# TrondVQ/UncertaintyQuantification-SleepApnea-1DCNN

Hardware: AMD Instinct MI355X
Metric: 30s-windows/sec for MCD T=50 & DE M=8 inference at 1/2/4/8 MI355X (higher is better)
Workload: dtype fp32; 1 GPU; global_batch=16384, seq_len=60, parallelism=dp1, mcd_passes=50, de_members=8, bn_mode_mcd=batch

## Files before the change

### uncertaintyquantification_sleepapnea_1dcnn_amd/csrc/x3_bindings.cpp

```cpp
#include <ATen/ATen.h>
#include <c10/core/DeviceGuard.h>
#include <c10/hip/HIPStream.h>
#include <torch/library.h>

#include <hip/hip_runtime_api.h>

#include "x3_args.h"

namespace apneauq {
int x3_lds_bytes(int layer);
int x3_tile_samples(int layer);
int x3_wg_per_cu(int layer);
hipError_t x3_launch_layer(int layer, const x3::LayerArgs& A, int grid, hipStream_t stream);
hipError_t x3_launch_l1(const x3::L1Args& A, hipStream_t stream);
hipError_t x3_launch_aff(const x3::AffArgs& A, hipStream_t stream);
hipError_t x3_launch_head(const x3::HeadArgs& A, hipStream_t stream);
}

namespace {

constexpr int kCh[7] = {4, 128, 192, 224, 96, 256, 96};
constexpr int kKs[6] = {7, 5, 3, 7, 9, 9};

inline hipStream_t cur_stream() { return c10::hip::getCurrentHIPStream().stream(); }
inline void check(hipError_t e, const char* what) { TORCH_CHECK(e == hipSuccess, what, " failed: ", hipGetErrorString(e)); }

inline void need(const at::Tensor& t, at::ScalarType dt, int64_t min_numel, const char* what) {
  TORCH_CHECK(t.is_cuda() && t.scalar_type() == dt && t.is_contiguous(), what, ": contiguous GPU tensor of dtype ", dt,
              " required");
  TORCH_CHECK(t.numel() >= min_numel, what, ": ", t.numel(), " elements, need >= ", min_numel);
  TORCH_CHECK(reinterpret_cast<uintptr_t>(t.data_ptr()) % 16 == 0, what, ": 16-B alignment required");
}

int num_cus(const at::Tensor& t) {
  int n = 0;
  check(hipDeviceGetAttribute(&n, hipDeviceAttributeMultiprocessorCount, t.device().index()), "hipDeviceGetAttribute");
  return n > 0 ? n : 256;
}

void x3_layer(int64_t layer, const at::Tensor& in, at::Tensor& out, const at::Tensor& wfrag, int64_t w_gstride,
              const at::Tensor& bias, const at::Tensor& wscale, int64_t p_gstride, const at::Tensor& aff_in,
              int64_t aff_gstride, const c10::optional<at::Tensor>& stats, int64_t n_win, int64_t groups,
              bool in_shared, int64_t thr_in, int64_t thr_out, int64_t seed, int64_t pass_base,
              int64_t window_offset, int64_t grid, const c10::optional<at::Tensor>& smax_in,
              const c10::optional<at::Tensor>& amax_in, const c10::optional<at::Tensor>& smax_out,
              const c10::optional<at::Tensor>& gscale_in, bool sign_in, bool sign_out) {
  TORCH_CHECK(layer >= 1 && layer <= 5, "x3_layer: layer must be 1..5 (block 2..6)");
  TORCH_CHECK(n_win >= 1 && groups >= 1, "x3_layer: empty launch");
  const int cin = kCh[layer], cout = kCh[layer + 1], ks = kKs[layer];
  const int64_t samples = n_win * groups, samples_in = in_shared ? n_win : samples;
  const int ts = apneauq::x3_tile_samples((int)layer);
  const int64_t tpg = (n_win + ts - 1) / ts;
  TORCH_CHECK(tpg * groups < (int64_t(1) << 31), "x3_layer: too many tiles");
  const int64_t wgroups = w_gstride ? groups : 1, pgroups = p_gstride ? groups : 1;
  need(in, at::kFloat, samples_in * 60 * cin, "x3_layer: in");
  need(out, at::kFloat, layer == 5 ? samples * 2 * cout : samples * 60 * cout, "x3_layer: out");
  const int64_t frag = (int64_t)(cin / 32) * ks * (cout / 16) * 128;
  TORCH_CHECK(w_gstride == 0 || w_gstride == frag, "x3_layer: w_gstride must be 0 or ", frag);
  need(wfrag, at::kHalf, wgroups * frag * 8, "x3_layer: wfrag");
  TORCH_CHECK(p_gstride == 0 || p_gstride == cout, "x3_layer: p_gstride must be 0 or ", cout);
  need(bias, at::kFloat, pgroups * cout, "x3_layer: bias");
  need(wscale, at::kFloat, pgroups, "x3_layer: wscale");
  TORCH_CHECK(aff_gstride == 0 || aff_gstride == 2 * cin, "x3_layer: aff_gstride must be 0 or ", 2 * cin);
  need(aff_in, at::kFloat, (aff_gstride ? groups : 1) * 2 * cin, "x3_layer: aff_in");
  double* st = nullptr;
  if (stats.has_value()) {
    need(*stats, at::kDouble, groups * apneauq::x3::kStatSlots * 2 * cout, "x3_layer: stats");
    st = stats->data_ptr<double>();
  }
  TORCH_CHECK(thr_in >= 0 && thr_in <= 65536 && thr_out >= 0 && thr_out <= 65536, "x3_layer: thresholds");
  const bool pre = smax_in.has_value() && smax_in->defined();
  TORCH_CHECK(pre == (amax_in.has_value() && amax_in->defined()), "x3_layer: smax_in and amax_in go together");
  if (pre) {
    need(*smax_in, at::kInt, samples_in, "x3_layer: smax_in");
    need(*amax_in, at::kFloat, (aff_gstride ? groups : 1) * 2, "x3_layer: amax_in");
  }
  const bool gpre = gscale_in.has_value() && gscale_in->defined();
  TORCH_CHECK(!(pre && gpre), "x3_layer: per-sample and per-group prescale are exclusive");
  if (gpre) need(*gscale_in, at::kFloat, aff_gstride ? groups : 1, "x3_layer: gscale_in");
  unsigned* smo = nullptr;
  if (smax_out.has_value() && smax_out->defined()) {
    TORCH_CHECK(layer < 5, "x3_layer: block 6 feeds the fp32 head (no smax_out)");
    need(*smax_out, at::kInt, samples, "x3_layer: smax_out");
    smo = reinterpret_cast<unsigned*>(smax_out->data_ptr<int>());
  }
  const at::DeviceGuard guard(in.device());
  apneauq::x3::LayerArgs A;
  A.in = in.data_ptr<float>();
  A.out = out.data_ptr<float>();
  A.wfrag = wfrag.data_ptr();
  A.w_gstride = w_gstride;
  A.bias = bias.data_ptr<float>();
  A.wscale = wscale.data_ptr<float>();
  A.p_gstride = (int)p_gstride;
  A.aff_in = aff_in.data_ptr<float>();
  A.aff_gstride = (int)aff_gstride;
  A.stats = st;
  A.smax_in = pre ? reinterpret_cast<const unsigned*>(smax_in->data_ptr<int>()) : nullptr;
  A.amax_in = pre ? amax_in->data_ptr<float>() : nullptr;
  A.smax_out = smo;
  A.gscale_in = gpre ? gscale_in->data_ptr<float>() : nullptr;
  A.n_win = (int)n_win;
  A.groups = (int)groups;
  A.tiles_per_group = (int)tpg;
  A.total_tiles = (int)(tpg * groups);
  A.in_shared = in_shared ? 1 : 0;
  TORCH_CHECK(!(sign_in && in_shared), "x3_layer: the shared block-1 output carries no masks");
  TORCH_CHECK(!(sign_out && layer == 5), "x3_layer: block 6 reduces its masked output in place");
  A.sign_in = sign_in ? 1 : 0;
  A.sign_out = sign_out ? 1 : 0;
  A.thr_in = (unsigned)thr_in;
  A.thr_out = (unsigned)thr_out;
  A.layer = (int)layer;
  A.pass_base = (unsigned)pass_base;
  A.window_offset = (unsigned)window_offset;
  A.seed = (unsigned long long)seed;
  int g = grid > 0 ? (int)grid : num_cus(in) * apneauq::x3_wg_per_cu((int)layer);
  if (g > A.total_tiles) g = A.total_tiles;
  check(apneauq::x3_launch_layer((int)layer, A, g, cur_stream()), "x3_layer");
}

void x3_l1(const at::Tensor& x, const at::Tensor& w, const at::Tensor& b, at::Tensor& out,
           const c10::optional<at::Tensor>& stats, int64_t n_win, int64_t groups, const c10::optional<at::Tensor>& smax) {
  TORCH_CHECK(n_win >= 1 && groups >= 1, "x3_l1: empty launch");
  need(x, at::kFloat, n_win * 60 * 4, "x3_l1: x");
  need(w, at::kFloat, groups * 7 * 4 * 128, "x3_l1: w");
  need(b, at::kFloat, groups * 128, "x3_l1: b");
  need(out, at::kFloat, groups * n_win * 60 * 128, "x3_l1: out");
  double* st = nullptr;
  if (stats.has_value()) {
    need(*stats, at::kDouble, groups * apneauq::x3::kStatSlots * 2 * 128, "x3_l1: stats");
    st = stats->data_ptr<double>();
  }
  unsigned* smp = nullptr;
  if (smax.has_value() && smax->defined()) {
    need(*smax, at::kInt, groups * n_win, "x3_l1: smax");
    smp = reinterpret_cast<unsigned*>(smax->data_ptr<int>());
  }
  const int64_t bpg = (n_win + apneauq::x3::kL1Win - 1) / apneauq::x3::kL1Win;
  TORCH_CHECK(bpg * groups < (int64_t(1) << 31), "x3_l1: too many blocks");
  const at::DeviceGuard guard(x.device());
  apneauq::x3::L1Args A{x.data_ptr<float>(), w.data_ptr<float>(), b.data_ptr<float>(), out.data_ptr<float>(), st, smp,
                        (int)n_win, (int)groups, (int)bpg};
  check(apneauq::x3_launch_l1(A, cur_stream()), "x3_l1");
}

void x3_aff(const c10::optional<at::Tensor>& stats, const at::Tensor& gamma, const at::Tensor& beta, at::Tensor& mmean,
            at::Tensor& mvar, at::Tensor& aff, int64_t C, int64_t groups, int64_t p_gstride, bool update,
            int64_t repeat, double inv_count, double eps, double momentum, double dsc,
            const c10::optional<at::Tensor>& amax, const c10::optional<at::Tensor>& gscale, bool running) {
  TORCH_CHECK(C >= 1 && C <= 4096 && groups >= 1, "x3_aff: bad sizes");
  TORCH_CHECK(!(running && update), "x3_aff: running affine and the moving update are exclusive");
  TORCH_CHECK(p_gstride == 0 || p_gstride == C, "x3_aff: p_gstride must be 0 or C");
  const int64_t pg = p_gstride ? groups : 1;
  need(gamma, at::kFloat, pg * C, "x3_aff: gamma");
  need(beta, at::kFloat, pg * C, "x3_aff: beta");
  need(mmean, at::kFloat, pg * C, "x3_aff: moving_mean");
  need(mvar, at::kFloat, pg * C, "x3_aff: moving_variance");
  need(aff, at::kFloat, groups * 2 * C, "x3_aff: aff");
  const double* st = nullptr;
  if (stats.has_value()) {
    need(*stats, at::kDouble, groups * apneauq::x3::kStatSlots * 2 * C, "x3_aff: stats");
    st = stats->data_ptr<double>();
  }
  TORCH_CHECK(!update || st != nullptr, "x3_aff: the moving update needs batch moments");
  float* amp = nullptr;
  if (amax.has_value() && amax->defined()) {
    need(*amax, at::kFloat, groups * 2, "x3_aff: amax");
    amp = amax->data_ptr<float>();
  }
  float* gsp = nullptr;
  if (gscale.has_value() && gscale->defined()) {
    TORCH_CHECK(st != nullptr && amp == nullptr, "x3_aff: gscale needs batch moments and excludes amax");
    need(*gscale, at::kFloat, groups, "x3_aff: gscale");
    gsp = gscale->data_ptr<float>();
  }
  const at::DeviceGuard guard(gamma.device());
  apneauq::x3::AffArgs A{st, gamma.data_ptr<float>(), beta.data_ptr<float>(), mmean.data_ptr<float>(),
                         mvar.data_ptr<float>(), aff.data_ptr<float>(), amp, gsp, (int)C, (int)groups, (int)p_gstride,
                         update ? 1 : 0, (int)repeat, inv_count, (float)eps, (float)momentum, (float)dsc,
                         running ? 1 : 0};
  check(apneauq::x3_launch_aff(A, cur_stream()), "x3_aff");
}

void x3_head(const at::Tensor& sums, const at::Tensor& aff, int64_t aff_gstride, const at::Tensor& dw,
             const at::Tensor& db, int64_t p_gstride, at::Tensor& out, int64_t n_win, int64_t groups, bool logits) {
  const int C = kCh[6];
  const int64_t samples = n_win * groups;
  TORCH_CHECK(samples >= 1 && samples < (int64_t(1) << 31), "x3_head: bad sample count");
  TORCH_CHECK(aff_gstride == 0 || aff_gstride == 2 * C, "x3_head: aff_gstride");
  TORCH_CHECK(p_gstride == 0 || p_gstride == C, "x3_head: p_gstride");
  need(sums, at::kFloat, samples * 2 * C, "x3_head: sums");
  need(aff, at::kFloat, (aff_gstride ? groups : 1) * 2 * C, "x3_head: aff");
  need(dw, at::kFloat, (p_gstride ? groups : 1) * C, "x3_head: dense w");
  need(db, at::kFloat, p_gstride ? groups : 1, "x3_head: dense b");
  need(out, at::kFloat, samples, "x3_head: out");
  const at::DeviceGuard guard(sums.device());
  apneauq::x3::HeadArgs A{sums.data_ptr<float>(), aff.data_ptr<float>(), dw.data_ptr<float>(), db.data_ptr<float>(),
                          out.data_ptr<float>(), C, (int)n_win, (int)samples, (int)aff_gstride, (int)p_gstride,
                          logits ? 1 : 0};
  check(apneauq::x3_launch_head(A, cur_stream()), "x3_head");
}

int64_t x3_lds(int64_t layer) { return apneauq::x3_lds_bytes((int)layer); }

}

TORCH_LIBRARY_FRAGMENT(apneauq, m) {
  m.def("x3_layer(int layer, Tensor input, Tensor(a!) out, Tensor wfrag, int w_gstride, Tensor bias, Tensor wscale, "
        "int p_gstride, Tensor aff_in, int aff_gstride, Tensor(b!)? stats, int n_win, int groups, bool in_shared, "
        "int thr_in, int thr_out, int seed, int pass_base, int window_offset, int grid, Tensor? smax_in=None, "
        "Tensor? amax_in=None, Tensor(c!)? smax_out=None, Tensor? gscale_in=None, bool sign_in=False, bool sign_out=False) -> ()");
  m.def("x3_l1(Tensor x, Tensor w, Tensor b, Tensor(a!) out, Tensor(b!)? stats, int n_win, int groups, "
        "Tensor(c!)? smax=None) -> ()");
  m.def("x3_aff(Tensor? stats, Tensor gamma, Tensor beta, Tensor(a!) mmean, Tensor(b!) mvar, Tensor(c!) aff, int C, "
        "int groups, int p_gstride, bool update, int repeat, float inv_count, float eps, float momentum, float dsc, "
        "Tensor(d!)? amax=None, Tensor(e!)? gscale=None, bool running=False) -> ()");
  m.def("x3_head(Tensor sums, Tensor aff, int aff_gstride, Tensor dw, Tensor db, int p_gstride, Tensor(a!) out, "
        "int n_win, int groups, bool logits) -> ()");
  m.def("x3_lds(int layer) -> int", &x3_lds);
}

TORCH_LIBRARY_IMPL(apneauq, CUDA, m) {
  m.impl("x3_layer", &x3_layer);
  m.impl("x3_l1", &x3_l1);
  m.impl("x3_head", &x3_head);
  m.impl("x3_aff", &x3_aff);
}
```

### uncertaintyquantification_sleepapnea_1dcnn_amd/csrc/x3_layers.hip

```cpp
#include "common.h"
#include "x3_args.h"

namespace apneauq {
namespace x3 {

typedef _Float16 f16x8 __attribute__((ext_vector_type(8)));
typedef _Float16 f16x4 __attribute__((ext_vector_type(4)));
typedef _Float16 f16x2 __attribute__((ext_vector_type(2)));
typedef __attribute__((address_space(1))) const f16x8 gf16x8;

constexpr int kStagers = 4;
constexpr int kL = 60, kSR = 64, kHalo = 4;
__host__ __device__ constexpr int row_bytes(int ck) { return 4 * ck + 32; }
__device__ __forceinline__ int sample_prescale(unsigned rmax_bits, const float* amax) {
  const float b = __builtin_fmaf(amax[0], __uint_as_float(rmax_bits), amax[1]);
  int e = 0;
  if (b > 0.f && b < INFINITY) frexpf(b, &e);
  return min(100, max(-100, 14 - e));
}

__host__ __device__ constexpr int lds_rows(int S) { return kHalo + S * kSR + kHalo; }
__host__ __device__ constexpr int buf_bytes(int S, int ck) { return lds_rows(S) * row_bytes(ck); }
__host__ __device__ constexpr int lds_bytes(int S, int cout, int ck) {
  return 2 * buf_bytes(S, ck) + 2 * cout * 8 + 2 * S * 4;
}

template <typename T>
__device__ __forceinline__ T gld(const void* p) {
  return *(const __attribute__((address_space(1))) T*)(p);
}

__device__ __forceinline__ int opaque_tid() {
  int t = threadIdx.x;
  asm volatile("" : "+v"(t));
  return t;
}

__device__ __forceinline__ f32x4 mfma(const f16x8& a, const f16x8& b, const f32x4& c) {
  return __builtin_amdgcn_mfma_f32_16x16x32_f16(a, b, c, 0, 0, 0);
}

__device__ __forceinline__ void lds_barrier() {
  __builtin_amdgcn_fence(__ATOMIC_RELEASE, "workgroup", "local");
  __builtin_amdgcn_s_barrier();
  __builtin_amdgcn_fence(__ATOMIC_ACQUIRE, "workgroup", "local");
}

__device__ __forceinline__ int xcd_wg() {
  const int nwg = gridDim.x, bid = blockIdx.x;
  const int q = nwg / 8, rem = nwg % 8, xcd = bid % 8;
  return (xcd < rem ? xcd * (q + 1) : rem * (q + 1) + (xcd - rem) * q) + bid / 8;
}

template <int NW, int WPC>
constexpr int waves_per_eu() { return NW * WPC > 8 ? (NW * WPC + 3) / 4 : NW * WPC <= 4 ? 1 : 2; }
constexpr int loaders(int lw) { return lw > 0 ? lw : 0; }
template <int CIN, int COUT, int KS, int S, int WM, int WN, bool LAST, int LW, int CK, int WPC, bool PS>
__global__ __launch_bounds__((WM * WN + loaders(LW)) * 64, (waves_per_eu<WM * WN + loaders(LW), WPC>())) void layer_kernel(
    const LayerArgs A) {
  extern __shared__ __attribute__((aligned(16))) char smem[];
  constexpr int NWM = WM * WN, NW = NWM + loaders(LW), kThreads = NW * 64;
  constexpr int kCK = CK, kRowB = row_bytes(CK), NQ = CK / 32, kQ = CK / 4;
  constexpr int kS = S, kBufB = buf_bytes(S, CK), kValidRows = S * kL, kUnits = kValidRows * kQ;
  constexpr int SW = LW > 0 ? LW : LW < 0 ? (-LW < NW ? -LW : NW) : (kStagers < NW ? kStagers : NW);
  constexpr int kSBase = LW > 0 ? NWM * 64 : 0;
  constexpr int kST = SW * 64;
  constexpr int kNU = (kUnits + kST - 1) / kST;
  static_assert(kST % kQ == 0 && (CK == 32 || CK == 64), "a staging thread keeps one channel quad");
  constexpr int NCH = CIN / kCK, NCTA = COUT / 16, NCT = NCTA / WN, NRT = 4 * S / WM, PAD = (KS - 1) / 2;
  constexpr int NSTEP = NCH * NQ * KS;
  constexpr int RG = NCT >= 4                        ? 1
                     : (NCT >= 3 && NCT * NRT > 16)    ? 1
                     : NCT == 1                        ? 4
                                                       : 2;
  constexpr bool BDB = NCT * NRT <= 24 && RG < 4;
  static_assert(NRT % RG == 0, "row-tile groups");
  constexpr long long FRAG_STEP = (long long)NCTA * 128;
  static_assert(CIN % kCK == 0 && COUT % 16 == 0, "channel tiling");
  static_assert(NCTA % WN == 0 && (4 * S) % WM == 0, "wave tiling");
  static_assert(NRT % 4 == 0, "whole 64-row sample slots per wave row (epilogue keys, block 6 sums)");
  double* st = reinterpret_cast<double*>(smem + 2 * kBufB);
  float* wsc = reinterpret_cast<float*>(smem + 2 * kBufB + 2 * COUT * 8);

  const int tid = threadIdx.x, lane = tid & 63;
  const int wave = __builtin_amdgcn_readfirstlane(tid >> 6);
  const int wn = wave % WN, wm = (wave / WN) % WM;
  const int ct0 = wn * NCT, rt0 = wm * NRT;
  const int m = lane & 15, h = lane >> 4;
  APNEAUQ_DASSERT(blockDim.x == kThreads);

  for (int i = tid; i < 2 * kBufB / 16; i += kThreads) reinterpret_cast<f32x4*>(smem)[i] = f32x4{0.f, 0.f, 0.f, 0.f};
  for (int i = tid; i < 2 * COUT; i += kThreads) st[i] = 0.0;
  __syncthreads();

  const int wg = xcd_wg();
  const int tpg = (A.n_win + S - 1) / S;
  const int total_tiles = tpg * A.groups;
  const int t_begin = (int)((long long)wg * total_tiles / gridDim.x);
  const int t_end = (int)((long long)(wg + 1) * total_tiles / gridDim.x);
  if (t_begin >= t_end) return;
  const int slot = wg % kStatSlots;

  const bool loader = LW > 0 && wave >= NWM;
  const bool stager = LW > 0 ? loader : wave < SW;
  struct Stage {
    f32x4 v[kNU];
    f32x4 a, b;
  };
  Stage s0;
  const bool hash_in = A.thr_in != 0u && !A.sign_in;
  const bool sign_in = A.thr_in != 0u && A.sign_in;
  const bool prescale = PS && A.smax_in != nullptr;
  int key_tile = -1;
  unsigned skeys[kS];
  unsigned skey_tile = 0u;
  static_assert(kS <= 8, "packed per-sample exponents");
  constexpr int kSP = (kS + 3) / 4;
  unsigned sa_pack[kSP];
  auto load_chunk = [&](int tile, int c, Stage& R) {
    const int tid = opaque_tid() - kSBase, q = tid % kQ;
    const int g = tile / tpg;
    const int w0 = (tile - g * tpg) * kS;
    const float* af = A.aff_in + (long long)g * A.aff_gstride + c * kCK + 4 * q;
    R.a = gld<f32x4>(af);
    R.b = gld<f32x4>(af + CIN);
#pragma unroll
    for (int u = 0; u < kNU; ++u) {
      const int ri = tid / kQ + (kST / kQ) * u;
      R.v[u] = f32x4{-0.f, -0.f, -0.f, -0.f};
      if (ri < kValidRows) {
        const int s = ri / kL, t = ri - s * kL, w = w0 + s;
        if (w < A.n_win) {
          const long long si = A.in_shared ? w : (long long)g * A.n_win + w;
          R.v[u] = gld<f32x4>(A.in + (si * kL + t) * CIN + c * kCK + 4 * q);
        }
      }
    }
  };
  auto store_chunk = [&](int tile, int c, char* buf, const Stage& R) {
    const int tid = opaque_tid() - kSBase, q = tid % kQ;
    const int g = tile / tpg;
    const int w0 = (tile - g * tpg) * kS;
    if (tile != key_tile) {
      const unsigned skey = stream_key(A.seed, A.layer - 1, A.pass_base + g);
      skey_tile = skey;
      const float* am = A.amax_in + (A.aff_gstride ? 2 * g : 0);
      float ws0 = A.wscale[A.p_gstride ? g : 0];
      if (A.gscale_in != nullptr) ws0 *= A.gscale_in[A.aff_gstride ? g : 0];
#pragma unroll
      for (int i = 0; i < kSP; ++i) sa_pack[i] = 0u;
#pragma unroll
      for (int s = 0; s < kS; ++s) {
        skeys[s] = sample_key(skey, A.window_offset + w0 + s);
        int sa = 0;
        if (prescale && w0 + s < A.n_win) {
          const long long si = A.in_shared ? w0 + s : (long long)g * A.n_win + w0 + s;
          sa = sample_prescale(A.smax_in[si], am);
          sa_pack[s >> 2] |= ((unsigned)sa & 0xFFu) << (8 * (s & 3));
        }
        if (tid == s) wsc[(tile & 1) * kS + s] = ldexpf(ws0, -sa);
      }
      key_tile = tile;
    }
#pragma unroll
    for (int u = 0; u < kNU; ++u) {
      const int ri = tid / kQ + (kST / kQ) * u;
      if (ri >= kValidRows) continue;
      const int s = ri / kL, t = ri - s * kL, w = w0 + s;
      const f32x4 v = R.v[u];
      bool keep[4];
      if (hash_in) {
        unsigned k;
        if constexpr (!PS) {
          k = sample_key(skey_tile, A.window_offset + w);
        } else {
          k = skeys[0];
#pragma unroll
          for (int j = 1; j < kS; ++j) k = s == j ? skeys[j] : k;
        }
        const unsigned b01 = dropout_bits2(k, t, c * kCK + 4 * q);
        const unsigned b23 = dropout_bits2(k, t, c * kCK + 4 * q + 2);
        keep[0] = (b01 & 0xFFFFu) >= A.thr_in;
        keep[1] = (b01 >> 16) >= A.thr_in;
        keep[2] = (b23 & 0xFFFFu) >= A.thr_in;
        keep[3] = (b23 >> 16) >= A.thr_in;
      } else if (sign_in) {
#pragma unroll
        for (int i = 0; i < 4; ++i) keep[i] = !__builtin_signbit(v[i]);
      } else {
#pragma unroll
        for (int i = 0; i < 4; ++i) keep[i] = true;
      }
      const bool valid = w < A.n_win;
      int sa = 0;
      if (prescale) {
        unsigned sp = sa_pack[0];
#pragma unroll
        for (int i = 1; i < kSP; ++i) sp = (s >> 2) == i ? sa_pack[i] : sp;
        sa = __builtin_amdgcn_sbfe((int)sp, 8 * (s & 3), 8);
      }
      float a[4];
#pragma unroll
      for (int i = 0; i < 4; ++i) a[i] = (valid && keep[i]) ? ldexpf(__builtin_fmaf(v[i], R.a[i], R.b[i]), sa) : 0.f;
      uint2 hi, lo;
#pragma unroll
      for (int p = 0; p < 2; ++p) {
        const unsigned u = __builtin_bit_cast(unsigned, (f16x2){(_Float16)a[2 * p], (_Float16)a[2 * p + 1]});
        unsigned l;
        asm("v_fma_mixlo_f16 %0, %1, -1.0, %2 op_sel_hi:[1,0,0]" : "=v"(l) : "v"(u), "v"(a[2 * p]));
        asm("v_fma_mixhi_f16 %0, %1, -1.0, %2 op_sel:[1,0,0] op_sel_hi:[1,0,0]"
                     : "+v"(l)
                     : "v"(u), "v"(a[2 * p + 1]));
        (p ? hi.y : hi.x) = u;
        (p ? lo.y : lo.x) = l;
      }
      char* row = buf + (kHalo + s * kSR + t) * kRowB + 8 * q;
      *reinterpret_cast<uint2*>(row) = hi;
      *reinterpret_cast<uint2*>(row + 2 * kCK) = lo;
    }
  };

  f32x4 acc[NCT][NRT];
#pragma unroll
  for (int ct = 0; ct < NCT; ++ct)
#pragma unroll
    for (int rt = 0; rt < NRT; ++rt) acc[ct][rt] = f32x4{0.f, 0.f, 0.f, 0.f};
  auto wbase = [&](int tile) -> const gf16x8* {
    const int g = tile / tpg;
    return (const gf16x8*)(A.wfrag) + (long long)g * A.w_gstride + ct0 * 128 + lane;
  };
  f16x8 ah[NCT], al[NCT];
  auto load_a = [&](const gf16x8* p, f16x8 (&xh)[NCT], f16x8 (&xl)[NCT]) {
#pragma unroll
    for (int ct = 0; ct < NCT; ++ct) {
      xh[ct] = p[ct * 128];
      xl[ct] = p[ct * 128 + 64];
    }
  };

  const int bofs = ((rt0 * 16 + m + kHalo - PAD) * kRowB) + 16 * h;

  auto compute_chunk = [&](int c, const char* buf, const gf16x8* wcur, const gf16x8* wnxt, auto&& hook) {
#pragma unroll
    for (int kk = 0; kk < NQ * KS; ++kk) {
      const int q2 = kk / KS, j = kk - q2 * KS;
      const char* bb = buf + bofs + q2 * 64;
      const int s = c * NQ * KS + kk;
      const gf16x8* np = (s + 1 < NSTEP) ? wcur + (long long)(s + 1) * FRAG_STEP : wnxt;
      f16x8 nh[NCT], nl[NCT];
      load_a(np, nh, nl);
      __builtin_amdgcn_sched_barrier(0);
      auto ldb = [&](int rt, f16x8& h_, f16x8& l_) {
        h_ = *reinterpret_cast<const f16x8*>(bb + (rt * 16 + j) * kRowB);
        l_ = *reinterpret_cast<const f16x8*>(bb + (rt * 16 + j) * kRowB + 2 * kCK);
      };
      f16x8 bh[RG], bl[RG];
#pragma unroll
      for (int r = 0; r < RG; ++r) ldb(r, bh[r], bl[r]);
#pragma unroll
      for (int rg = 0; rg < NRT; rg += RG) {
        f16x8 bh2[RG], bl2[RG];
#pragma unroll
        for (int r = 0; r < RG; ++r) {
          bh2[r] = bh[r];
          bl2[r] = bl[r];
          if (BDB && rg + RG < NRT) ldb(rg + RG + r, bh2[r], bl2[r]);
          if (!BDB) ldb(rg + r, bh[r], bl[r]);
        }
        __builtin_amdgcn_sched_barrier(0);
#pragma unroll
        for (int r = 0; r < RG; ++r)
#pragma unroll
          for (int ct = 0; ct < NCT; ++ct) acc[ct][rg + r] = mfma(ah[ct], bh[r], acc[ct][rg + r]);
#pragma unroll
        for (int r = 0; r < RG; ++r)
#pragma unroll
          for (int ct = 0; ct < NCT; ++ct) acc[ct][rg + r] = mfma(al[ct], bh[r], acc[ct][rg + r]);
#pragma unroll
        for (int r = 0; r < RG; ++r)
#pragma unroll
          for (int ct = 0; ct < NCT; ++ct) acc[ct][rg + r] = mfma(ah[ct], bl[r], acc[ct][rg + r]);
#pragma unroll
        for (int r = 0; r < RG; ++r) {
          bh[r] = bh2[r];
          bl[r] = bl2[r];
        }
      }
#pragma unroll
      for (int ct = 0; ct < NCT; ++ct) {
        ah[ct] = nh[ct];
        al[ct] = nl[ct];
      }
      __builtin_amdgcn_sched_barrier(0);
      if (kk == (NQ * KS) / 2) hook();
    }
  };

  auto epilogue = [&](int tile) {
    const int lane = opaque_tid() & 63, m = lane & 15, h = lane >> 4;
    const int g = tile / tpg;
    const int w0 = (tile - g * tpg) * kS;
    float wsq[NRT / 4];
#pragma unroll
    for (int q = 0; q < NRT / 4; ++q) wsq[q] = wsc[(tile & 1) * kS + (rt0 >> 2) + q];
    const bool track = PS && !LAST && A.smax_out != nullptr;
    float mxs[NRT / 4];
#pragma unroll
    for (int q = 0; q < NRT / 4; ++q) mxs[q] = 0.f;
    const float* bias = A.bias + (long long)g * A.p_gstride;
    const bool drop = (LAST || A.sign_out) && A.thr_out != 0u;
    unsigned skeys[NRT / 4];
    if (drop) {
      const unsigned skey = stream_key(A.seed, A.layer, A.pass_base + g);
#pragma unroll
      for (int q = 0; q < NRT / 4; ++q)
        skeys[q] = sample_key(skey, A.window_offset + w0 + (rt0 >> 2) + q);
    }
#pragma unroll
    for (int ct = 0; ct < NCT; ++ct) {
      const int co0 = (ct0 + ct) * 16 + 4 * h;
      const f32x4 b4 = gld<f32x4>(bias + co0);
      f32x4 s1 = {0.f, 0.f, 0.f, 0.f}, s2 = s1, k1 = s1, k0 = s1;
#pragma unroll
      for (int rt = 0; rt < NRT; ++rt) {
        const int s = (rt0 + rt) >> 2, t = (((rt0 + rt) & 3) << 4) + m, w = w0 + s;
        const bool valid = t < kL && w < A.n_win;
        f32x4 r;
#pragma unroll
        for (int e = 0; e < 4; ++e) r[e] = fmaxf(__builtin_fmaf(acc[ct][rt][e], wsq[rt >> 2], b4[e]), 0.f);
        acc[ct][rt] = f32x4{0.f, 0.f, 0.f, 0.f};
        bool keep[4] = {true, true, true, true};
        if (drop) {
          const unsigned key = skeys[rt >> 2];
          const unsigned b01 = dropout_bits2(key, t, co0), b23 = dropout_bits2(key, t, co0 + 2);
          keep[0] = (b01 & 0xFFFFu) >= A.thr_out;
          keep[1] = (b01 >> 16) >= A.thr_out;
          keep[2] = (b23 & 0xFFFFu) >= A.thr_out;
          keep[3] = (b23 >> 16) >= A.thr_out;
        }
        if (valid) {
#pragma unroll
          for (int e = 0; e < 4; ++e) {
            s1[e] += r[e];
            s2[e] = __builtin_fmaf(r[e], r[e], s2[e]);
            if (!LAST) mxs[rt >> 2] = fmaxf(mxs[rt >> 2], r[e]);
            if constexpr (LAST) {
              k1[e] += keep[e] ? r[e] : 0.f;
              k0[e] += keep[e] ? 1.f : 0.f;
            }
          }
          if constexpr (!LAST) {
            const long long sample = (long long)g * A.n_win + w;
            f32x4 o = r;
            if (drop) {
#pragma unroll
              for (int e = 0; e < 4; ++e) o[e] = keep[e] ? r[e] : __builtin_copysignf(r[e], -1.f);
            }
            *reinterpret_cast<f32x4*>(A.out + (sample * kL + t) * COUT + co0) = o;
          }
        }
        if constexpr (LAST) {
          if ((rt & 3) == 3) {
#pragma unroll
            for (int e = 0; e < 4; ++e) {
              k1[e] = group16_sum(k1[e]);
              k0[e] = group16_sum(k0[e]);
            }
            const int wl = w0 + (rt0 + rt) / 4;
            if (m == 0 && wl < A.n_win) {
              float* o = A.out + ((long long)g * A.n_win + wl) * (2 * COUT);
              *reinterpret_cast<f32x4*>(o + co0) = k1;
              *reinterpret_cast<f32x4*>(o + COUT + co0) = k0;
            }
            k1 = f32x4{0.f, 0.f, 0.f, 0.f};
            k0 = k1;
          }
        }
      }
      if (A.stats != nullptr) {
#pragma unroll
        for (int e = 0; e < 4; ++e) {
          const float a = group16_sum(s1[e]), b = group16_sum(s2[e]);
          if (m == 0) {
            atomicAdd(&st[co0 + e], (double)a);
            atomicAdd(&st[COUT + co0 + e], (double)b);
          }
        }
      }
    }
    if (track) {
#pragma unroll
      for (int q = 0; q < NRT / 4; ++q) {
        const float mq = wave_max(mxs[q]);
        const int w = w0 + (rt0 >> 2) + q;
        if (lane == 0 && w < A.n_win) atomicMax(A.smax_out + (long long)g * A.n_win + w, __float_as_uint(mq));
      }
    }
  };

  auto flush_stats = [&](int g) {
    __syncthreads();
    if (A.stats != nullptr) {
      double* dst = A.stats + ((long long)g * kStatSlots + slot) * 2 * COUT;
      for (int i = tid; i < 2 * COUT; i += kThreads) {
        atomicAdd(dst + i, st[i]);
        st[i] = 0.0;
      }
    }
    __syncthreads();
  };

  const int total = (t_end - t_begin) * NCH;
  auto chunk_tile = [&](int it) { return t_begin + it / NCH; };
  int g_cur = t_begin / tpg;
  if constexpr (LW > 0) {
    if (loader) {
      if (stager) {
        load_chunk(t_begin, 0, s0);
        store_chunk(t_begin, 0, smem, s0);
      }
      lds_barrier();
      if (stager && total > 1) load_chunk(chunk_tile(1), 1 % NCH, s0);
#pragma unroll 1
      for (int it = 0; it < total; ++it) {
        const int tile = chunk_tile(it), c = it - (tile - t_begin) * NCH;
        if (c == 0) {
          const int g = tile / tpg;
          if (g != g_cur) {
            flush_stats(g_cur);
            g_cur = g;
          }
        }
        if (stager && it + 1 < total) store_chunk(chunk_tile(it + 1), (it + 1) % NCH, smem + ((it + 1) & 1) * kBufB, s0);
        lds_barrier();
        if (stager && it + 2 < total) load_chunk(chunk_tile(it + 2), (it + 2) % NCH, s0);
      }
      flush_stats(g_cur);
      return;
    }
    lds_barrier();
    load_a(wbase(t_begin), ah, al);
#pragma unroll 1
    for (int it = 0; it < total; ++it) {
      const int tile = chunk_tile(it), c = it - (tile - t_begin) * NCH;
      if (c == 0) {
        const int g = tile / tpg;
        if (g != g_cur) {
          flush_stats(g_cur);
          g_cur = g;
        }
      }
      const gf16x8* wcur = wbase(tile);
      const gf16x8* wnxt = wbase(tile + 1 < t_end ? tile + 1 : tile);
      compute_chunk(c, smem + (it & 1) * kBufB, wcur, wnxt, []() {});
      if (c == NCH - 1) epilogue(tile);
      lds_barrier();
    }
    flush_stats(g_cur);
    return;
  }
  if (stager) {
    load_chunk(t_begin, 0, s0);
    store_chunk(t_begin, 0, smem, s0);
  }
  lds_barrier();
  if (stager && total > 1) load_chunk(chunk_tile(1), 1 % NCH, s0);
  load_a(wbase(t_begin), ah, al);
#pragma unroll 1
  for (int it = 0; it < total; ++it) {
    const int tile = chunk_tile(it), c = it - (tile - t_begin) * NCH;
    if (c == 0) {
      const int g = tile / tpg;
      if (g != g_cur) {
        flush_stats(g_cur);
        g_cur = g;
      }
    }
    const gf16x8* wcur = wbase(tile);
    const gf16x8* wnxt = wbase(tile + 1 < t_end ? tile + 1 : tile);
    char* buf = smem + (it & 1) * kBufB;
    char* nbuf = smem + ((it + 1) & 1) * kBufB;
    compute_chunk(c, buf, wcur, wnxt, [&]() {
      if (stager && it + 1 < total) store_chunk(chunk_tile(it + 1), (it + 1) % NCH, nbuf, s0);
    });
    if (c == NCH - 1) epilogue(tile);
    lds_barrier();
    if (stager && it + 2 < total) load_chunk(chunk_tile(it + 2), (it + 2) % NCH, s0);
  }
  flush_stats(g_cur);
}

__global__ __launch_bounds__(256) void l1_kernel(const L1Args A) {
  __shared__ float xs[kL1Win][kL + 6][4];
  __shared__ float red[2][2][128];
  __shared__ unsigned wmax[kL1Win];
  const int g = blockIdx.x / A.blocks_per_group;
  const int w0 = (blockIdx.x - g * A.blocks_per_group) * kL1Win;
  const int tid = threadIdx.x, c = tid & 127, half = tid >> 7;
  for (int i = tid; i < kL1Win * (kL + 6) * 4; i += 256) {
    const int s = i / ((kL + 6) * 4), r = (i / 4) % (kL + 6), ci = i & 3;
    const int t = r - 3, w = w0 + s;
    xs[s][r][ci] = (t >= 0 && t < kL && w < A.n_win) ? A.x[((long long)w * kL + t) * 4 + ci] : 0.f;
  }
  float wr[7][4];
#pragma unroll
  for (int j = 0; j < 7; ++j)
#pragma unroll
    for (int ci = 0; ci < 4; ++ci) wr[j][ci] = A.w[(((long long)g * 7 + j) * 4 + ci) * 128 + c];
  const float bc = A.b[g * 128 + c];
  if (tid < kL1Win) wmax[tid] = 0u;
  __syncthreads();
  float s1 = 0.f, s2 = 0.f;
  for (int s = 0; s < kL1Win; ++s) {
    const int w = w0 + s;
    if (w >= A.n_win) break;
    float* o = A.out + (((long long)g * A.n_win + w) * kL) * 128 + c;
    float mx = 0.f;
    for (int t = half * 30; t < half * 30 + 30; ++t) {
      float v = bc;
#pragma unroll
      for (int j = 0; j < 7; ++j)
#pragma unroll
        for (int ci = 0; ci < 4; ++ci) v = __builtin_fmaf(xs[s][t + j][ci], wr[j][ci], v);
      v = fmaxf(v, 0.f);
      o[t * 128] = v;
      s1 += v;
      s2 = __builtin_fmaf(v, v, s2);
      mx = fmaxf(mx, v);
    }
    if (A.smax != nullptr) {
      mx = wave_max(mx);
      if ((tid & 63) == 0) atomicMax(&wmax[s], __float_as_uint(mx));
    }
  }
  if (A.stats != nullptr || A.smax != nullptr) {
    red[half][0][c] = s1;
    red[half][1][c] = s2;
    __syncthreads();
    if (A.stats != nullptr && tid < 128) {
      double* dst = A.stats + ((long long)g * kStatSlots + (blockIdx.x % kStatSlots)) * 2 * 128;
      atomicAdd(dst + c, (double)red[0][0][c] + (double)red[1][0][c]);
      atomicAdd(dst + 128 + c, (double)red[0][1][c] + (double)red[1][1][c]);
    }
    if (A.smax != nullptr && tid < kL1Win && w0 + tid < A.n_win) A.smax[(long long)g * A.n_win + w0 + tid] = wmax[tid];
  }
}

__device__ __forceinline__ void aff_moments(const AffArgs& A, int g, int c, float& mean, float& var) {
  const double* p = A.stats + (long long)g * kStatSlots * 2 * A.C + c;
  double a = 0.0, b = 0.0;
#pragma unroll
  for (int s = 0; s < kStatSlots; ++s) {
    a += p[s * 2 * A.C];
    b += p[s * 2 * A.C + A.C];
  }
  const double mu = a * A.inv_count;
  mean = (float)mu;
  var = (float)fmax(b * A.inv_count - mu * mu, 0.0);
}

__global__ __launch_bounds__(256) void aff_kernel(const AffArgs A) {
  __shared__ float red[2][4];
  const int tid = threadIdx.x;
  if ((int)blockIdx.x == A.groups) {
    for (int c = tid; c < A.C; c += 256)
      for (int g = 0; g < A.groups; ++g) {
        const long long po = (long long)g * A.p_gstride + c;
        float mean, var;
        aff_moments(A, g, c, mean, var);
        for (int r = 0; r < A.repeat; ++r) {
          A.mmean[po] = A.mmean[po] * A.momentum + mean * (1.f - A.momentum);
          A.mvar[po] = A.mvar[po] * A.momentum + var * (1.f - A.momentum);
        }
      }
    return;
  }
  {
    const int g = blockIdx.x;
    float ms = 0.f, mt = 0.f;
    for (int c = tid; c < A.C; c += 256) {
      const long long po = (long long)g * A.p_gstride + c;
      float mean, var;
      if (A.stats != nullptr && !A.running) {
        aff_moments(A, g, c, mean, var);
      } else {
        mean = A.mmean[po];
        var = A.mvar[po];
      }
      const float sc = A.gamma[po] / sqrtf(var + A.eps);
      const float s_ = sc * A.dsc, t_ = (A.beta[po] - mean * sc) * A.dsc;
      A.aff[((long long)g * 2) * A.C + c] = s_;
      A.aff[((long long)g * 2 + 1) * A.C + c] = t_;
      if (A.gscale != nullptr) {
        const double* p = A.stats + (long long)g * kStatSlots * 2 * A.C + A.C + c;
        double q = 0.0;
        for (int s = 0; s < kStatSlots; ++s) q += p[s * 2 * A.C];
        ms = fmaxf(ms, __builtin_fmaf(fabsf(s_), (float)sqrt(fmax(q, 0.0)) * 1.0001f, fabsf(t_)));
      } else {
        ms = fmaxf(ms, fabsf(s_));
        mt = fmaxf(mt, fabsf(t_));
      }
    }
    if (A.gscale != nullptr) {
      ms = wave_max(ms);
      if ((tid & 63) == 0) red[0][tid >> 6] = ms;
      __syncthreads();
      const float bnd = fmaxf(fmaxf(red[0][0], red[0][1]), fmaxf(red[0][2], red[0][3]));
      int e = 0;
      if (bnd > 0.f && bnd < INFINITY) frexpf(bnd, &e);
      const int sa = min(100, max(-100, 14 - e));
      for (int c = tid; c < A.C; c += 256) {
        float* af = A.aff + (long long)g * 2 * A.C + c;
        af[0] = ldexpf(af[0], sa);
        af[A.C] = ldexpf(af[A.C], sa);
      }
      if (tid == 0) A.gscale[g] = ldexpf(1.f, -sa);
      return;
    }
    if (A.amax == nullptr) return;
    ms = wave_max(ms);
    mt = wave_max(mt);
    if ((tid & 63) == 0) {
      red[0][tid >> 6] = ms;
      red[1][tid >> 6] = mt;
    }
    __syncthreads();
    if (tid == 0) {
      A.amax[2 * g] = fmaxf(fmaxf(red[0][0], red[0][1]), fmaxf(red[0][2], red[0][3]));
      A.amax[2 * g + 1] = fmaxf(fmaxf(red[1][0], red[1][1]), fmaxf(red[1][2], red[1][3]));
    }
  }
}

__global__ __launch_bounds__(256) void head_kernel(const HeadArgs A) {
  const int lane = threadIdx.x & 63;
  const long long sidx = (long long)blockIdx.x * 4 + (threadIdx.x >> 6);
  if (sidx >= A.samples) return;
  const int g = (int)(sidx / A.n_win);
  const float* s = A.sums + sidx * 2 * A.C;
  const float* af = A.aff + (long long)g * A.aff_gstride;
  const float* dw = A.dw + (long long)g * A.p_gstride;
  float v = 0.f;
  for (int c = lane; c < A.C; c += 64) v += dw[c] * __builtin_fmaf(af[c], s[c], af[A.C + c] * s[A.C + c]);
  v = wave_sum(v);
  if (lane == 0) {
    const float logit = v * (1.0f / kL) + A.db[A.p_gstride ? g : 0];
    A.out[sidx] = A.out_logits ? logit : 1.0f / (1.0f + expf(-logit));
  }
}

template <int CIN, int COUT, int KS, int S, int WM, int WN, bool LAST, int LW, int CK, int WPC, bool PS>
hipError_t launch_layer(const LayerArgs& A, int grid, hipStream_t stream) {
  constexpr int lds = lds_bytes(S, COUT, CK);
  static_assert(WPC * lds <= 160 * 1024, "LDS of the workgroups sharing a CU");
  auto k = layer_kernel<CIN, COUT, KS, S, WM, WN, LAST, LW, CK, WPC, PS>;
  static bool attr = false;
  if (!attr) {
    hipError_t e = hipFuncSetAttribute(reinterpret_cast<const void*>(k), hipFuncAttributeMaxDynamicSharedMemorySize, lds);
    if (e != hipSuccess) return e;
    attr = true;
  }
  hipLaunchKernelGGL(k, dim3(grid), dim3((WM * WN + loaders(LW)) * 64), lds, stream, A);
  return hipGetLastError();
}

}

#ifdef APNEAUQ_X3_TABLE
#include APNEAUQ_X3_TABLE
#else
#define APNEAUQ_X3_LAYERS(X)                     \
  X(1, 128, 192, 5, 4, 2, 4, false, -8, 0, 32, 1) \
  X(2, 192, 224, 3, 2, 1, 7, false, 4, 4, 64, 1) \
  X(3, 224, 96, 7, 4, 2, 2, false, 4, 4, 32, 1)  \
  X(4, 96, 256, 9, 2, 1, 8, false, 4, 4, 32, 1)  \
  X(5, 256, 96, 9, 4, 2, 2, true, 4, 4, 64, 1)
#endif

int x3_lds_bytes(int layer) {
#define APNEAUQ_X3_LDS(L, CI, CO, K, S, WM, WN, LAST, LW, LWB, CK, WPC) \
  if (layer == L) return x3::lds_bytes(S, CO, CK);
  APNEAUQ_X3_LAYERS(APNEAUQ_X3_LDS)
#undef APNEAUQ_X3_LDS
  return 0;
}

int x3_tile_samples(int layer) {
#define APNEAUQ_X3_TS(L, CI, CO, K, S, WM, WN, LAST, LW, LWB, CK, WPC) \
  if (layer == L) return S;
  APNEAUQ_X3_LAYERS(APNEAUQ_X3_TS)
#undef APNEAUQ_X3_TS
  return 0;
}

int x3_wg_per_cu(int layer) {
#define APNEAUQ_X3_WPC(L, CI, CO, K, S, WM, WN, LAST, LW, LWB, CK, WPC) \
  if (layer == L) return WPC;
  APNEAUQ_X3_LAYERS(APNEAUQ_X3_WPC)
#undef APNEAUQ_X3_WPC
  return 1;
}

hipError_t x3_launch_layer(int layer, const x3::LayerArgs& A, int grid, hipStream_t stream) {
  using namespace x3;
  const bool ps = A.smax_in != nullptr || A.smax_out != nullptr;
#define APNEAUQ_X3_LAUNCH(L, CI, CO, K, S, WM, WN, LAST, LW, LWB, CK, WPC)                                  \
  if (layer == L) {                                                                                       \
    return ps ? launch_layer<CI, CO, K, S, WM, WN, LAST, LW, CK, WPC, true>(A, grid, stream)               \
              : launch_layer<CI, CO, K, S, WM, WN, LAST, LWB, CK, WPC, false>(A, grid, stream);            \
  }
  APNEAUQ_X3_LAYERS(APNEAUQ_X3_LAUNCH)
#undef APNEAUQ_X3_LAUNCH
  return hipErrorInvalidValue;
}

hipError_t x3_launch_l1(const x3::L1Args& A, hipStream_t stream) {
  const int grid = A.groups * A.blocks_per_group;
  if (grid <= 0) return hipSuccess;
  hipLaunchKernelGGL(x3::l1_kernel, dim3(grid), dim3(256), 0, stream, A);
  return hipGetLastError();
}

hipError_t x3_launch_aff(const x3::AffArgs& A, hipStream_t stream) {
  const int blocks = A.groups + (A.stats != nullptr && A.update ? 1 : 0);
  hipLaunchKernelGGL(x3::aff_kernel, dim3(blocks), dim3(256), 0, stream, A);
  return hipGetLastError();
}

hipError_t x3_launch_head(const x3::HeadArgs& A, hipStream_t stream) {
  if (A.samples <= 0) return hipSuccess;
  hipLaunchKernelGGL(x3::head_kernel, dim3((A.samples + 3) / 4), dim3(256), 0, stream, A);
  return hipGetLastError();
}

}
```

### uncertaintyquantification_sleepapnea_1dcnn_amd/ops/x3.py

```python
from __future__ import annotations

import math
import os
from typing import Callable, Dict, List, Optional, Sequence

import torch

from ..models.spec import ModelSpec
from . import _ext, fused, rng

CH = fused.FUSED_CHANNELS
KS = fused.FUSED_KSIZES
STAT_SLOTS = 16
TILE = 4
CK = 32
BYTES_PER_SAMPLE = 60 * (192 + 256) * 4
R1_BYTES = 60 * 128 * 4


def supports(spec: ModelSpec) -> bool:
    return fused.supports(spec)


def pack_conv(kernel: torch.Tensor):
    k, cin, cout = kernel.shape
    assert cin % CK == 0 and cout % 16 == 0
    w = kernel.detach().to(torch.float64)
    amax = float(w.abs().max()) if w.numel() else 0.0
    sw = 13 - math.frexp(amax)[1] + 1 if amax > 0 else 0
    ws = (w * (2.0 ** sw)).float()
    hi = ws.half()
    lo = (ws - hi.float()).half()
    nch, nct = cin // CK, cout // 16

    def frag(p):
        v = p.reshape(k, nch, 4, 8, nct, 16)
        return v.permute(1, 0, 4, 2, 5, 3).reshape(nch, k, nct, 64, 8)

    fr = torch.stack([frag(hi), frag(lo)], dim=3)
    return fr.contiguous().reshape(-1), 2.0 ** (-sw)


def unpack_conv(fr: torch.Tensor, wscale: float, k: int, cin: int, cout: int) -> torch.Tensor:
    nch, nct = cin // CK, cout // 16
    v = fr.reshape(nch, k, nct, 2, 4, 16, 8).float()
    w = v[:, :, :, 0] + v[:, :, :, 1]
    w = w.permute(1, 0, 3, 5, 2, 4).reshape(k, cin, cout)
    return w.double().mul(wscale).float()


class X3Model:

    def __init__(self, spec: ModelSpec, params: Sequence[Dict[str, torch.Tensor]], device=None):
        if not supports(spec):
            raise ValueError("the x3 engine implements the reference (60, 4) no-pool architecture")
        self.spec = spec
        self.G = len(params)
        dev = torch.device(device) if device is not None else params[0]["conv1d_1/kernel"].device
        if dev.type == "cuda" and dev.index is None:
            dev = torch.device("cuda", torch.cuda.current_device())
        self.device = dev
        f32 = dict(dtype=torch.float32, device=dev)
        self.w1 = torch.stack([p["conv1d_1/kernel"].to(**f32) for p in params]).contiguous()
        self.b1 = torch.stack([p["conv1d_1/bias"].to(**f32) for p in params]).contiguous()
        self.wfrag: List[Optional[torch.Tensor]] = [None]
        self.wscale: List[Optional[torch.Tensor]] = [None]
        self.bias: List[torch.Tensor] = [self.b1]
        for l in range(1, 6):
            frs, scs = [], []
            for p in params:
                fr, sc = pack_conv(p[f"conv1d_{l + 1}/kernel"].to(dev))
                frs.append(fr)
                scs.append(sc)
            self.wfrag.append(torch.stack(frs).contiguous())
            self.wscale.append(torch.tensor(scs, **f32))
            self.bias.append(torch.stack([p[f"conv1d_{l + 1}/bias"].to(**f32) for p in params]).contiguous())
        self.bn = []
        for l in range(6):
            names = [f"batchnorm_{l + 1}/{n}" for n in ("gamma", "beta", "moving_mean", "moving_variance")]
            entry = []
            for n in names:
                src = params[0][n]
                if self.G == 1 and src.device == dev and src.dtype == torch.float32 and src.is_contiguous():
                    entry.append(src.view(1, -1))
                else:
                    entry.append(torch.stack([p[n].to(**f32) for p in params]).contiguous())
            self.bn.append(entry)
        self.dw = torch.stack([p["output_layer/kernel"].to(**f32).reshape(-1) for p in params]).contiguous()
        self.db = torch.stack([p["output_layer/bias"].to(**f32).reshape(-1) for p in params]).reshape(-1).contiguous()
        self._ws: Dict[tuple, "_Workspace"] = {}

    def workspace(self, samples: int, n_r1: int, groups: int) -> "_Workspace":
        ws = self._ws.get("ws")
        if ws is None or ws.samples < samples or ws.n_r1 < n_r1 or ws.groups < groups:
            self._ws.clear()
            ws = self._ws["ws"] = _Workspace(self.device, samples, n_r1, groups)
        return ws


class _Workspace:
    def __init__(self, dev, samples: int, n_r1: int, groups: int):
        self.samples, self.n_r1, self.groups = int(samples), int(n_r1), max(int(groups), 1)
        f32 = dict(dtype=torch.float32, device=dev)
        self.r1 = torch.empty(n_r1 * 60 * CH[1], **f32)
        self.buf = [torch.empty(samples * 60 * 192, **f32), torch.empty(samples * 60 * 256, **f32)]
        self.sums = torch.empty(samples * 2 * CH[6], **f32)
        self.out = torch.empty(samples, **f32)
        self.stats = [torch.zeros(max(groups, 1) * STAT_SLOTS * 2 * CH[l + 1], dtype=torch.float64, device=dev)
                      for l in range(6)]
        self.aff = [torch.empty(max(groups, 1) * 2 * CH[l + 1], **f32) for l in range(6)]
        self.smax = [torch.zeros(n_r1 if l == 0 else samples, dtype=torch.int32, device=dev) for l in range(5)]
        self.amax = [torch.zeros(max(groups, 1) * 2, **f32) for l in range(6)]
        self.gscale = [torch.ones(max(groups, 1), **f32) for l in range(5)] + [None]

    def smax_out(self, l: int, k: int) -> Optional[torch.Tensor]:
        if l >= 5:
            return None
        return self.smax[l][:k].zero_()


def _ops():
    return _ext.ops()


_SIGN_DEFAULT = "2,4"


def _sign_layers() -> frozenset:
    v = os.environ.get("APNEAUQ_X3_SIGN_MASK", _SIGN_DEFAULT)
    return frozenset(int(t) for t in v.replace(" ", "").split(",") if t)


def _sign(l: int, sl: frozenset):
    return (l - 1) in sl and l >= 2, l in sl and l <= 4


def _dsc(rate: float) -> float:
    return 1.0 / (1.0 - rate) if rate < 1.0 else 0.0


def _sync_stats(sync: Callable, st: torch.Tensor, groups: int, c: int) -> None:
    v = st[: groups * STAT_SLOTS * 2 * c].view(groups, STAT_SLOTS, 2 * c)
    tot = v.sum(1)
    sync(tot)
    v.zero_()
    v[:, 0].copy_(tot)


def _max_samples(dev, per_sample: int, frac: float = 0.45) -> int:
    import os

    free = torch.cuda.mem_get_info(dev)[0]
    cap = float(os.environ.get("APNEAUQ_X3_WS_GB", "20")) * 2 ** 30
    return max(1, int(min(free * frac, cap)) // per_sample)


@torch.no_grad()
def mcd_batch(model: X3Model, x: torch.Tensor, n_pass: int, seed: int, pass_base: int = 0, window_offset: int = 0,
              update_moving: bool = True, sync: Optional[Callable] = None, global_n: Optional[int] = None,
              max_samples: Optional[int] = None, grid: int = 0) -> torch.Tensor:
    assert model.G == 1, "mcd_batch runs one model"
    spec, o = model.spec, _ops()
    x = x.to(device=model.device, dtype=torch.float32).contiguous()
    n = x.shape[0]
    gn = int(global_n or n)
    if max_samples is None:
        max_samples = _max_samples(model.device, BYTES_PER_SAMPLE + R1_BYTES)
        if sync is not None:
            t = torch.tensor([float(max_samples)], dtype=torch.float64, device=model.device)
            import torch.distributed as dist

            from ..parallel import comm

            comm.run("chunking_all_reduce_min", t, lambda: dist.all_reduce(t, op=dist.ReduceOp.MIN))
            max_samples = int(t.item())
    ref_n = n
    if sync is not None and global_n:
        import torch.distributed as dist

        w = dist.get_world_size() if dist.is_initialized() else 1
        ref_n = -(-gn // w)
    if ref_n > max_samples:
        return _mcd_batch_windowed(model, x, n_pass, seed, pass_base, window_offset, update_moving, sync, gn,
                                   max_samples)
    cap = max(1, min(n_pass, max_samples // max(ref_n, 1)))
    n_chunks = -(-n_pass // cap)
    chunk = -(-n_pass // n_chunks)
    ws = model.workspace(chunk * n, n, chunk)
    inv_count = 1.0 / (gn * 60.0)
    thr = [rng.dropout_threshold(b.dropout) for b in spec.blocks]
    dsc = [_dsc(b.dropout) for b in spec.blocks]
    eps, mom = float(spec.bn_epsilon), float(spec.bn_momentum)
    seed = int(seed) & ((1 << 63) - 1)
    sl = _sign_layers()
    out = torch.empty(n_pass, n, dtype=torch.float32, device=model.device)
    ws.stats[0].zero_()
    o.x3_l1(x, model.w1, model.b1, ws.r1, ws.stats[0], n, 1, None)
    if sync is not None:
        _sync_stats(sync, ws.stats[0], 1, CH[1])
    g, b, mm, mv = model.bn[0]
    o.x3_aff(ws.stats[0], g, b, mm, mv, ws.aff[0], CH[1], 1, 0, bool(update_moving), n_pass, inv_count, eps, mom, dsc[0],
             None, ws.gscale[0])
    for t0 in range(0, n_pass, chunk):
        tc = min(chunk, n_pass - t0)
        pb = int(pass_base) + t0
        for l in range(1, 6):
            c = CH[l + 1]
            st = ws.stats[l]
            st[: tc * STAT_SLOTS * 2 * c].zero_()
            src = ws.r1 if l == 1 else ws.buf[(l - 2) % 2]
            dst = ws.sums if l == 5 else ws.buf[(l - 1) % 2]
            o.x3_layer(l, src, dst, model.wfrag[l], 0, model.bias[l], model.wscale[l], 0, ws.aff[l - 1],
                       0 if l == 1 else 2 * CH[l], st, n, tc, l == 1, thr[l - 1], thr[l], seed, pb,
                       int(window_offset), int(grid), None, None, None, ws.gscale[l - 1], *_sign(l, sl))
            if sync is not None:
                _sync_stats(sync, st, tc, c)
            g, b, mm, mv = model.bn[l]
            o.x3_aff(st, g, b, mm, mv, ws.aff[l], c, tc, 0, bool(update_moving), 1, inv_count, eps, mom, dsc[l],
                     None, ws.gscale[l])
        o.x3_head(ws.sums, ws.aff[5], 2 * CH[6], model.dw, model.db, 0, ws.out, n, tc, False)
        out[t0: t0 + tc].copy_(ws.out[: tc * n].view(tc, n))
    return out


def _mcd_batch_windowed(model: X3Model, x: torch.Tensor, n_pass: int, seed: int, pass_base: int,
                        window_offset: int, update_moving: bool, sync: Optional[Callable], gn: int,
                        max_samples: int) -> torch.Tensor:
    spec, o = model.spec, _ops()
    n = x.shape[0]
    wc = max(1, int(max_samples))
    bounds = [(s, min(n, s + wc)) for s in range(0, n, wc)]
    ws = model.workspace(wc, wc, 1)
    inv_count = 1.0 / (gn * 60.0)
    thr = [rng.dropout_threshold(b.dropout) for b in spec.blocks]
    dsc = [_dsc(b.dropout) for b in spec.blocks]
    eps, mom = float(spec.bn_epsilon), float(spec.bn_momentum)
    seed = int(seed) & ((1 << 63) - 1)
    sl = _sign_layers()
    out = torch.empty(n_pass, n, dtype=torch.float32, device=model.device)

    def run(s: int, e: int, upto: int, pb: int, stats_layer: int) -> None:
        m = e - s
        o.x3_l1(x[s:e], model.w1, model.b1, ws.r1, ws.stats[0] if stats_layer == 0 else None, m, 1, None)
        for l in range(1, upto + 1):
            src = ws.r1 if l == 1 else ws.buf[(l - 2) % 2]
            dst = ws.sums if l == 5 else ws.buf[(l - 1) % 2]
            o.x3_layer(l, src, dst, model.wfrag[l], 0, model.bias[l], model.wscale[l], 0, ws.aff[l - 1],
                       0 if l == 1 else 2 * CH[l], ws.stats[l] if l == stats_layer else None, m, 1, l == 1,
                       thr[l - 1], thr[l], seed, pb, int(window_offset) + s, 0, None, None, None, ws.gscale[l - 1],
                       *_sign(l, sl))

    def finish_layer(l: int, repeat: int) -> None:
        if sync is not None:
            _sync_stats(sync, ws.stats[l], 1, CH[l + 1])
        g, b, mm, mv = model.bn[l]
        o.x3_aff(ws.stats[l], g, b, mm, mv, ws.aff[l], CH[l + 1], 1, 0, bool(update_moving), repeat, inv_count, eps,
                 mom, dsc[l], None, ws.gscale[l])

    ws.stats[0].zero_()
    for s, e in bounds:
        run(s, e, 0, int(pass_base), 0)
    finish_layer(0, n_pass)
    for t in range(n_pass):
        pb = int(pass_base) + t
        for l in range(1, 6):
            ws.stats[l].zero_()
            for s, e in bounds:
                run(s, e, l, pb, l)
            finish_layer(l, 1)
        for s, e in bounds:
            run(s, e, 5, pb, -1)
            o.x3_head(ws.sums, ws.aff[5], 0, model.dw, model.db, 0, ws.out, e - s, 1, False)
            out[t, s:e].copy_(ws.out[: e - s])
    return out


@torch.no_grad()
def forward_running(model: X3Model, x: torch.Tensor, n_pass: int = 1, dropout: bool = False, seed: int = 0,
                    pass_offset: int = 0, window_offset: int = 0, logits: bool = False,
                    max_samples: Optional[int] = None) -> torch.Tensor:
    x = x.to(device=model.device, dtype=torch.float32).contiguous()
    n = x.shape[0]
    groups = (n_pass if dropout else model.G) if n > 0 else 1
    if max_samples is None:
        max_samples = _max_samples(model.device, BYTES_PER_SAMPLE + R1_BYTES)
    wc = max(1, int(max_samples) // max(groups, 1))
    if n <= wc:
        return _forward_running(model, x, n_pass, dropout, seed, pass_offset, window_offset, logits)
    parts = [_forward_running(model, x[s: s + wc], n_pass, dropout, seed, pass_offset, int(window_offset) + s, logits)
             for s in range(0, n, wc)]
    return torch.cat(parts, dim=2)


def _forward_running(model: X3Model, x: torch.Tensor, n_pass: int, dropout: bool, seed: int, pass_offset: int,
                     window_offset: int, logits: bool) -> torch.Tensor:
    spec, o = model.spec, _ops()
    n = x.shape[0]
    G = model.G
    if dropout and G != 1:
        raise ValueError("MC Dropout runs one model")
    if not dropout:
        n_pass = 1
    groups = n_pass if dropout else G
    ws = model.workspace(groups * n, n * G, max(groups, G))
    thr = [rng.dropout_threshold(b.dropout) if dropout else 0 for b in spec.blocks]
    dsc = [_dsc(b.dropout) if dropout else 1.0 for b in spec.blocks]
    eps, mom = float(spec.bn_epsilon), float(spec.bn_momentum)
    seed = int(seed) & ((1 << 63) - 1)
    if not dropout:
        return _predict_members(model, ws, x, G, eps, mom, logits)
    sl = _sign_layers()
    for l in range(6):
        g, b, mm, mv = model.bn[l]
        o.x3_aff(None, g, b, mm, mv, ws.aff[l], CH[l + 1], G, CH[l + 1] if G > 1 else 0, False, 1, 1.0, eps, mom,
                 dsc[l], ws.amax[l])
    o.x3_l1(x, model.w1, model.b1, ws.r1, None, n, G, ws.smax[0])
    per_member = G > 1
    for l in range(1, 6):
        src = ws.r1 if l == 1 else ws.buf[(l - 2) % 2]
        dst = ws.sums if l == 5 else ws.buf[(l - 1) % 2]
        wstride = model.wfrag[l].shape[1] // 8 if per_member else 0
        sm = ws.smax_out(l, groups * n)
        o.x3_layer(l, src, dst, model.wfrag[l], wstride, model.bias[l], model.wscale[l],
                   CH[l + 1] if per_member else 0, ws.aff[l - 1], 2 * CH[l] if per_member else 0, None, n, groups,
                   dropout and l == 1, thr[l - 1], thr[l], seed, int(pass_offset),
                   int(window_offset), 0, ws.smax[l - 1], ws.amax[l - 1], sm, None, *_sign(l, sl))
    o.x3_head(ws.sums, ws.aff[5], 2 * CH[6] if per_member else 0, model.dw, model.db, CH[6] if per_member else 0,
              ws.out, n, groups, bool(logits))
    return ws.out[: groups * n].view(G, n_pass, n).clone()


def _predict_members(model: X3Model, ws: "_Workspace", x: torch.Tensor, G: int, eps: float, mom: float,
                     logits: bool) -> torch.Tensor:
    spec, o = model.spec, _ops()
    n = x.shape[0]
    per_member = G > 1
    ps = CH[1:] if per_member else [0] * 6
    o.zero_buffers([ws.stats[l][: G * STAT_SLOTS * 2 * CH[l + 1]] for l in range(5)])
    g, b, mm, mv = model.bn[5]
    o.x3_aff(None, g, b, mm, mv, ws.aff[5], CH[6], G, ps[5], False, 1, 1.0, eps, mom, 1.0, None)
    o.x3_l1(x, model.w1, model.b1, ws.r1, ws.stats[0], n, G, None)
    for l in range(1, 6):
        g, b, mm, mv = model.bn[l - 1]
        o.x3_aff(ws.stats[l - 1], g, b, mm, mv, ws.aff[l - 1], CH[l], G, ps[l - 1], False, 1, 1.0, eps, mom, 1.0,
                 None, ws.gscale[l - 1], True)
        src = ws.r1 if l == 1 else ws.buf[(l - 2) % 2]
        dst = ws.sums if l == 5 else ws.buf[(l - 1) % 2]
        wstride = model.wfrag[l].shape[1] // 8 if per_member else 0
        o.x3_layer(l, src, dst, model.wfrag[l], wstride, model.bias[l], model.wscale[l], ps[l],
                   ws.aff[l - 1], 2 * CH[l] if per_member else 0, ws.stats[l] if l < 5 else None, n, G, False, 0, 0,
                   0, 0, 0, 0, None, None, None, ws.gscale[l - 1], False, False)
    o.x3_head(ws.sums, ws.aff[5], 2 * CH[6] if per_member else 0, model.dw, model.db, CH[6] if per_member else 0,
              ws.out, n, G, bool(logits))
    return ws.out[: G * n].view(G, 1, n).clone()


def split_f16(a: torch.Tensor):
    hi = a.half()
    lo = (a - hi.float()).half()
    return hi, lo


def emulate_conv(h: torch.Tensor, fr: torch.Tensor, wscale: float, k: int, cin: int, cout: int) -> torch.Tensor:
    from ..models.reference import conv1d_same

    nch, nct = cin // CK, cout // 16
    v = fr.reshape(nch, k, nct, 2, 4, 16, 8).double()
    whi = v[:, :, :, 0].permute(1, 0, 3, 5, 2, 4).reshape(k, cin, cout)
    wlo = v[:, :, :, 1].permute(1, 0, 3, 5, 2, 4).reshape(k, cin, cout)
    ah, al = split_f16(h.float())
    ah, al = ah.double(), al.double()
    z = torch.zeros(cout, dtype=torch.float64)
    y = conv1d_same(ah, whi, z) + conv1d_same(ah, wlo, z) + conv1d_same(al, whi, z)
    return y * wscale
```

Baseline: 62120 windows/s.

## Add dense-row tiling for conv blocks 2-5 that packs timesteps across window boundaries

Adds a dense-row variant of the conv layer kernel. Each tile covers a contiguous run of timestep rows across windows (64*S rows), instead of S whole 60-step windows padded to 64-row slots. This removes the wasted MFMA rows that come from padding each 60-step window to 64. The cost is extra staging of halo edges, per-row slot arithmetic, and more complex dropout key and mask handling in the epilogue. It is enabled by default for layers 1-4 in the batch-moment and ensemble paths.

```diff
diff --git a/uncertaintyquantification_sleepapnea_1dcnn_amd/csrc/x3_bindings.cpp b/uncertaintyquantification_sleepapnea_1dcnn_amd/csrc/x3_bindings.cpp
--- a/uncertaintyquantification_sleepapnea_1dcnn_amd/csrc/x3_bindings.cpp
+++ b/uncertaintyquantification_sleepapnea_1dcnn_amd/csrc/x3_bindings.cpp
@@ -6,12 +6,14 @@
 #include <hip/hip_runtime_api.h>
 
 #include "x3_args.h"
+#include "x3_dense_map.h"
 
 namespace apneauq {
 int x3_lds_bytes(int layer);
 int x3_tile_samples(int layer);
 int x3_wg_per_cu(int layer);
-hipError_t x3_launch_layer(int layer, const x3::LayerArgs& A, int grid, hipStream_t stream);
+bool x3_has_dense(int layer);
+hipError_t x3_launch_layer(int layer, const x3::LayerArgs& A, int grid, bool dense_rows, hipStream_t stream);
 hipError_t x3_launch_l1(const x3::L1Args& A, hipStream_t stream);
 hipError_t x3_launch_aff(const x3::AffArgs& A, hipStream_t stream);
 hipError_t x3_launch_head(const x3::HeadArgs& A, hipStream_t stream);
@@ -44,13 +46,16 @@
               bool in_shared, int64_t thr_in, int64_t thr_out, int64_t seed, int64_t pass_base,
               int64_t window_offset, int64_t grid, const c10::optional<at::Tensor>& smax_in,
               const c10::optional<at::Tensor>& amax_in, const c10::optional<at::Tensor>& smax_out,
-              const c10::optional<at::Tensor>& gscale_in, bool sign_in, bool sign_out) {
+              const c10::optional<at::Tensor>& gscale_in, bool sign_in, bool sign_out, bool dense_rows) {
   TORCH_CHECK(layer >= 1 && layer <= 5, "x3_layer: layer must be 1..5 (block 2..6)");
   TORCH_CHECK(n_win >= 1 && groups >= 1, "x3_layer: empty launch");
   const int cin = kCh[layer], cout = kCh[layer + 1], ks = kKs[layer];
   const int64_t samples = n_win * groups, samples_in = in_shared ? n_win : samples;
   const int ts = apneauq::x3_tile_samples((int)layer);
-  const int64_t tpg = (n_win + ts - 1) / ts;
+  TORCH_CHECK(!dense_rows || apneauq::x3_has_dense((int)layer), "x3_layer: layer ", layer,
+              " has no dense-row kernel");
+  TORCH_CHECK(!dense_rows || n_win < (int64_t(1) << 24), "x3_layer: too many windows for dense rows");
+  const int64_t tpg = dense_rows ? apneauq::x3::dense::tiles(n_win, 64 * ts) : (n_win + ts - 1) / ts;
   TORCH_CHECK(tpg * groups < (int64_t(1) << 31), "x3_layer: too many tiles");
   const int64_t wgroups = w_gstride ? groups : 1, pgroups = p_gstride ? groups : 1;
   need(in, at::kFloat, samples_in * 60 * cin, "x3_layer: in");
@@ -75,6 +80,8 @@
     need(*smax_in, at::kInt, samples_in, "x3_layer: smax_in");
     need(*amax_in, at::kFloat, (aff_gstride ? groups : 1) * 2, "x3_layer: amax_in");
   }
+  TORCH_CHECK(!(dense_rows && (pre || (smax_out.has_value() && smax_out->defined()))),
+              "x3_layer: the per-sample prescale kernels keep whole-window slots");
   const bool gpre = gscale_in.has_value() && gscale_in->defined();
   TORCH_CHECK(!(pre && gpre), "x3_layer: per-sample and per-group prescale are exclusive");
   if (gpre) need(*gscale_in, at::kFloat, aff_gstride ? groups : 1, "x3_layer: gscale_in");
@@ -117,7 +124,7 @@
   A.seed = (unsigned long long)seed;
   int g = grid > 0 ? (int)grid : num_cus(in) * apneauq::x3_wg_per_cu((int)layer);
   if (g > A.total_tiles) g = A.total_tiles;
-  check(apneauq::x3_launch_layer((int)layer, A, g, cur_stream()), "x3_layer");
+  check(apneauq::x3_launch_layer((int)layer, A, g, dense_rows, cur_stream()), "x3_layer");
 }
 
 void x3_l1(const at::Tensor& x, const at::Tensor& w, const at::Tensor& b, at::Tensor& out,
@@ -203,6 +210,7 @@
 }
 
 int64_t x3_lds(int64_t layer) { return apneauq::x3_lds_bytes((int)layer); }
+bool x3_has_dense(int64_t layer) { return apneauq::x3_has_dense((int)layer); }
 
 }
 
@@ -210,7 +218,8 @@
   m.def("x3_layer(int layer, Tensor input, Tensor(a!) out, Tensor wfrag, int w_gstride, Tensor bias, Tensor wscale, "
         "int p_gstride, Tensor aff_in, int aff_gstride, Tensor(b!)? stats, int n_win, int groups, bool in_shared, "
         "int thr_in, int thr_out, int seed, int pass_base, int window_offset, int grid, Tensor? smax_in=None, "
-        "Tensor? amax_in=None, Tensor(c!)? smax_out=None, Tensor? gscale_in=None, bool sign_in=False, bool sign_out=False) -> ()");
+        "Tensor? amax_in=None, Tensor(c!)? smax_out=None, Tensor? gscale_in=None, bool sign_in=False, bool sign_out=False, "
+        "bool dense_rows=False) -> ()");
   m.def("x3_l1(Tensor x, Tensor w, Tensor b, Tensor(a!) out, Tensor(b!)? stats, int n_win, int groups, "
         "Tensor(c!)? smax=None) -> ()");
   m.def("x3_aff(Tensor? stats, Tensor gamma, Tensor beta, Tensor(a!) mmean, Tensor(b!) mvar, Tensor(c!) aff, int C, "
@@ -219,6 +228,7 @@
   m.def("x3_head(Tensor sums, Tensor aff, int aff_gstride, Tensor dw, Tensor db, int p_gstride, Tensor(a!) out, "
         "int n_win, int groups, bool logits) -> ()");
   m.def("x3_lds(int layer) -> int", &x3_lds);
+  m.def("x3_has_dense(int layer) -> bool", &x3_has_dense);
 }
 
 TORCH_LIBRARY_IMPL(apneauq, CUDA, m) {
diff --git a/uncertaintyquantification_sleepapnea_1dcnn_amd/csrc/x3_dense_map.h b/uncertaintyquantification_sleepapnea_1dcnn_amd/csrc/x3_dense_map.h
--- /dev/null
+++ b/uncertaintyquantification_sleepapnea_1dcnn_amd/csrc/x3_dense_map.h
@@ -0,0 +1,41 @@
+#pragma once
+
+#ifndef __host__
+#define APNEAUQ_X3_DENSE_MAP_PLAIN 1
+#define __host__
+#define __device__
+#endif
+
+namespace apneauq {
+namespace x3 {
+namespace dense {
+
+constexpr int kLen = 60, kSlot = 64, kHaloRows = 4;
+
+__host__ __device__ constexpr long long tiles(long long n_win, int rows) { return (kLen * n_win + rows - 1) / rows; }
+__host__ __device__ constexpr int max_windows(int rows) { return (kLen - 4 + rows - 1) / kLen + 1; }
+__host__ __device__ constexpr int lds_rows(int rows) { return kHaloRows + kSlot * max_windows(rows) + kHaloRows; }
+
+__host__ __device__ constexpr long long first_row(long long tl, int rows) { return tl * rows; }
+__host__ __device__ constexpr int first_window(long long tl, int rows) { return (int)(first_row(tl, rows) / kLen); }
+__host__ __device__ constexpr int offset(long long tl, int rows) { return (int)(first_row(tl, rows) % kLen); }
+__host__ __device__ constexpr int windows(int off, int rows) { return (off + rows - 1) / kLen + 1; }
+
+__host__ __device__ constexpr int slot_of(int dl) { return (int)(((unsigned)dl & 1023u) * 1093u >> 16); }
+__host__ __device__ constexpr int step_of(int dl) { return dl - kLen * slot_of(dl); }
+__host__ __device__ constexpr int lds_row(int dl) { return kHaloRows + dl + (kSlot - kLen) * slot_of(dl); }
+
+__host__ __device__ constexpr int staged_units(int rows, int pad) { return rows + 2 * pad; }
+__host__ __device__ constexpr bool staged(int dl, int off, int rows, int pad) {
+  return dl >= 0 && dl >= off - pad && dl < off + rows + pad && dl < kLen * windows(off, rows);
+}
+
+}
+}
+}
+
+#ifdef APNEAUQ_X3_DENSE_MAP_PLAIN
+#undef __host__
+#undef __device__
+#undef APNEAUQ_X3_DENSE_MAP_PLAIN
+#endif
diff --git a/uncertaintyquantification_sleepapnea_1dcnn_amd/csrc/x3_layers.hip b/uncertaintyquantification_sleepapnea_1dcnn_amd/csrc/x3_layers.hip
--- a/uncertaintyquantification_sleepapnea_1dcnn_amd/csrc/x3_layers.hip
+++ b/uncertaintyquantification_sleepapnea_1dcnn_amd/csrc/x3_layers.hip
@@ -1,5 +1,6 @@
 #include "common.h"
 #include "x3_args.h"
+#include "x3_dense_map.h"
 
 namespace apneauq {
 namespace x3 {
@@ -21,8 +22,8 @@
 
 __host__ __device__ constexpr int lds_rows(int S) { return kHalo + S * kSR + kHalo; }
 __host__ __device__ constexpr int buf_bytes(int S, int ck) { return lds_rows(S) * row_bytes(ck); }
-__host__ __device__ constexpr int lds_bytes(int S, int cout, int ck) {
-  return 2 * buf_bytes(S, ck) + 2 * cout * 8 + 2 * S * 4;
+__host__ __device__ constexpr int lds_bytes(int S, int cout, int ck, bool dense_rows = false) {
+  return 2 * (dense_rows ? dense::lds_rows(kSR * S) * row_bytes(ck) : buf_bytes(S, ck)) + 2 * cout * 8 + 2 * S * 4;
 }
 
 template <typename T>
@@ -55,19 +56,24 @@
 template <int NW, int WPC>
 constexpr int waves_per_eu() { return NW * WPC > 8 ? (NW * WPC + 3) / 4 : NW * WPC <= 4 ? 1 : 2; }
 constexpr int loaders(int lw) { return lw > 0 ? lw : 0; }
-template <int CIN, int COUT, int KS, int S, int WM, int WN, bool LAST, int LW, int CK, int WPC, bool PS>
+template <int CIN, int COUT, int KS, int S, int WM, int WN, bool LAST, int LW, int CK, int WPC, bool PS, bool DENSE = false>
 __global__ __launch_bounds__((WM * WN + loaders(LW)) * 64, (waves_per_eu<WM * WN + loaders(LW), WPC>())) void layer_kernel(
     const LayerArgs A) {
   extern __shared__ __attribute__((aligned(16))) char smem[];
   constexpr int NWM = WM * WN, NW = NWM + loaders(LW), kThreads = NW * 64;
   constexpr int kCK = CK, kRowB = row_bytes(CK), NQ = CK / 32, kQ = CK / 4;
-  constexpr int kS = S, kBufB = buf_bytes(S, CK), kValidRows = S * kL, kUnits = kValidRows * kQ;
+  constexpr int PAD = (KS - 1) / 2, kRows = kSR * S;
+  static_assert(!DENSE || (!PS && !LAST), "dense rows: batch-moment blocks 2..5 only");
+  constexpr int kS = S, kBufB = DENSE ? dense::lds_rows(kRows) * kRowB : buf_bytes(S, CK);
+  constexpr int kValidRows = DENSE ? kRows : S * kL, kUnits = kValidRows * kQ;
   constexpr int SW = LW > 0 ? LW : LW < 0 ? (-LW < NW ? -LW : NW) : (kStagers < NW ? kStagers : NW);
   constexpr int kSBase = LW > 0 ? NWM * 64 : 0;
   constexpr int kST = SW * 64;
-  constexpr int kNU = (kUnits + kST - 1) / kST;
+  constexpr int kMainU = (kUnits + kST - 1) / kST, kNU = kMainU + (DENSE ? 1 : 0);
+  constexpr int kEdgeWaves = (2 * PAD * kQ + 63) / 64;
+  static_assert(!DENSE || (kUnits % kST == 0 && kEdgeWaves <= SW), "dense rows: whole staging steps per tile");
   static_assert(kST % kQ == 0 && (CK == 32 || CK == 64), "a staging thread keeps one channel quad");
-  constexpr int NCH = CIN / kCK, NCTA = COUT / 16, NCT = NCTA / WN, NRT = 4 * S / WM, PAD = (KS - 1) / 2;
+  constexpr int NCH = CIN / kCK, NCTA = COUT / 16, NCT = NCTA / WN, NRT = 4 * S / WM;
   constexpr int NSTEP = NCH * NQ * KS;
   constexpr int RG = NCT >= 4                        ? 1
                      : (NCT >= 3 && NCT * NRT > 16)    ? 1
@@ -94,7 +100,7 @@
   __syncthreads();
 
   const int wg = xcd_wg();
-  const int tpg = (A.n_win + S - 1) / S;
+  const int tpg = DENSE ? (int)dense::tiles(A.n_win, kRows) : (A.n_win + S - 1) / S;
   const int total_tiles = tpg * A.groups;
   const int t_begin = (int)((long long)wg * total_tiles / gridDim.x);
   const int t_end = (int)((long long)(wg + 1) * total_tiles / gridDim.x);
@@ -103,6 +109,16 @@
 
   const bool loader = LW > 0 && wave >= NWM;
   const bool stager = LW > 0 ? loader : wave < SW;
+  const bool edge_wave = DENSE && wave >= kSBase / 64 && wave - kSBase / 64 < kEdgeWaves;
+  auto dense_unit = [&](int u, int tid, int off, int& dl) -> bool {
+    const int r = tid / kQ;
+    if (u < kMainU) {
+      dl = off + r + (kST / kQ) * u;
+      return true;
+    }
+    dl = r < PAD ? off - PAD + r : off + kRows - PAD + r;
+    return edge_wave && r < 2 * PAD && dense::staged(dl, off, kRows, PAD);
+  };
   struct Stage {
     f32x4 v[kNU];
     f32x4 a, b;
@@ -120,7 +136,7 @@
   auto load_chunk = [&](int tile, int c, Stage& R) {
     const int tid = opaque_tid() - kSBase, q = tid % kQ;
     const int g = tile / tpg;
-    const int w0 = (tile - g * tpg) * kS;
+    const int w0 = (tile - g * tpg) * (DENSE ? kRows : kS);
     const float* af = A.aff_in + (long long)g * A.aff_gstride + c * kCK + 4 * q;
     R.a = gld<f32x4>(af);
     R.b = gld<f32x4>(af + CIN);
@@ -128,7 +144,14 @@
     for (int u = 0; u < kNU; ++u) {
       const int ri = tid / kQ + (kST / kQ) * u;
       R.v[u] = f32x4{-0.f, -0.f, -0.f, -0.f};
-      if (ri < kValidRows) {
+      if constexpr (DENSE) {
+        const int wf = w0 / kL, off = w0 - wf * kL;
+        int dl;
+        if (dense_unit(u, tid, off, dl) && wf + dense::slot_of(dl) < A.n_win) {
+          const long long r0 = (A.in_shared ? 0ll : (long long)g * A.n_win * kL) + wf * kL;
+          R.v[u] = gld<f32x4>(A.in + (r0 + dl) * CIN + c * kCK + 4 * q);
+        }
+      } else if (ri < kValidRows) {
         const int s = ri / kL, t = ri - s * kL, w = w0 + s;
         if (w < A.n_win) {
           const long long si = A.in_shared ? w : (long long)g * A.n_win + w;
@@ -140,7 +163,7 @@
   auto store_chunk = [&](int tile, int c, char* buf, const Stage& R) {
     const int tid = opaque_tid() - kSBase, q = tid % kQ;
     const int g = tile / tpg;
-    const int w0 = (tile - g * tpg) * kS;
+    const int w0 = (tile - g * tpg) * (DENSE ? kRows : kS);
     if (tile != key_tile) {
       const unsigned skey = stream_key(A.seed, A.layer - 1, A.pass_base + g);
       skey_tile = skey;
@@ -149,8 +172,9 @@
       if (A.gscale_in != nullptr) ws0 *= A.gscale_in[A.aff_gstride ? g : 0];
 #pragma unroll
       for (int i = 0; i < kSP; ++i) sa_pack[i] = 0u;
-#pragma unroll
-      for (int s = 0; s < kS; ++s) {
+      if (DENSE && tid == 0) wsc[(tile & 1) * kS] = ws0;
+#pragma unroll
+      for (int s = 0; s < (DENSE ? 0 : kS); ++s) {
         skeys[s] = sample_key(skey, A.window_offset + w0 + s);
         int sa = 0;
         if (prescale && w0 + s < A.n_win) {
@@ -165,8 +189,16 @@
 #pragma unroll
     for (int u = 0; u < kNU; ++u) {
       const int ri = tid / kQ + (kST / kQ) * u;
-      if (ri >= kValidRows) continue;
-      const int s = ri / kL, t = ri - s * kL, w = w0 + s;
+      int s, t, w, lrow;
+      if constexpr (DENSE) {
+        const int wf = w0 / kL, off = w0 - wf * kL;
+        int dl;
+        if (!dense_unit(u, tid, off, dl)) continue;
+        s = dense::slot_of(dl), t = dl - s * kL, w = wf + s, lrow = dense::lds_row(dl);
+      } else {
+        if (ri >= kValidRows) continue;
+        s = ri / kL, t = ri - s * kL, w = w0 + s, lrow = kHalo + s * kSR + t;
+      }
       const f32x4 v = R.v[u];
       bool keep[4];
       if (hash_in) {
@@ -214,7 +246,7 @@
         (p ? hi.y : hi.x) = u;
         (p ? lo.y : lo.x) = l;
       }
-      char* row = buf + (kHalo + s * kSR + t) * kRowB + 8 * q;
+      char* row = buf + lrow * kRowB + 8 * q;
       *reinterpret_cast<uint2*>(row) = hi;
       *reinterpret_cast<uint2*>(row + 2 * kCK) = lo;
     }
@@ -240,7 +272,13 @@
 
   const int bofs = ((rt0 * 16 + m + kHalo - PAD) * kRowB) + 16 * h;
 
-  auto compute_chunk = [&](int c, const char* buf, const gf16x8* wcur, const gf16x8* wnxt, auto&& hook) {
+  auto compute_chunk = [&](int c, int off, const char* buf, const gf16x8* wcur, const gf16x8* wnxt, auto&& hook) {
+    const char* bp[DENSE ? NRT : 1];
+    if constexpr (DENSE) {
+#pragma unroll
+      for (int rt = 0; rt < NRT; ++rt)
+        bp[rt] = buf + bofs + (off + (dense::kSlot - kL) * ((off + (rt0 + rt) * 16 + m) / kL)) * kRowB;
+    }
 #pragma unroll
     for (int kk = 0; kk < NQ * KS; ++kk) {
       const int q2 = kk / KS, j = kk - q2 * KS;
@@ -251,8 +289,9 @@
       load_a(np, nh, nl);
       __builtin_amdgcn_sched_barrier(0);
       auto ldb = [&](int rt, f16x8& h_, f16x8& l_) {
-        h_ = *reinterpret_cast<const f16x8*>(bb + (rt * 16 + j) * kRowB);
-        l_ = *reinterpret_cast<const f16x8*>(bb + (rt * 16 + j) * kRowB + 2 * kCK);
+        const char* br = DENSE ? bp[rt] + q2 * 64 : bb;
+        h_ = *reinterpret_cast<const f16x8*>(br + (rt * 16 + j) * kRowB);
+        l_ = *reinterpret_cast<const f16x8*>(br + (rt * 16 + j) * kRowB + 2 * kCK);
       };
       f16x8 bh[RG], bl[RG];
 #pragma unroll
@@ -299,39 +338,55 @@
   auto epilogue = [&](int tile) {
     const int lane = opaque_tid() & 63, m = lane & 15, h = lane >> 4;
     const int g = tile / tpg;
-    const int w0 = (tile - g * tpg) * kS;
+    const int w0 = (tile - g * tpg) * (DENSE ? kRows : kS);
     float wsq[NRT / 4];
 #pragma unroll
-    for (int q = 0; q < NRT / 4; ++q) wsq[q] = wsc[(tile & 1) * kS + (rt0 >> 2) + q];
+    for (int q = 0; q < NRT / 4; ++q) wsq[q] = wsc[(tile & 1) * kS + (DENSE ? 0 : (rt0 >> 2) + q)];
     const bool track = PS && !LAST && A.smax_out != nullptr;
     float mxs[NRT / 4];
 #pragma unroll
     for (int q = 0; q < NRT / 4; ++q) mxs[q] = 0.f;
     const float* bias = A.bias + (long long)g * A.p_gstride;
     const bool drop = (LAST || A.sign_out) && A.thr_out != 0u;
-    unsigned skeys[NRT / 4];
+    constexpr int NKEY = DENSE ? dense::max_windows(kRows) : NRT / 4;
+    const int wf = DENSE ? w0 / kL : 0, off = DENSE ? w0 - wf * kL : 0;
+    unsigned skeys[NKEY];
     if (drop) {
       const unsigned skey = stream_key(A.seed, A.layer, A.pass_base + g);
 #pragma unroll
-      for (int q = 0; q < NRT / 4; ++q)
-        skeys[q] = sample_key(skey, A.window_offset + w0 + (rt0 >> 2) + q);
+      for (int q = 0; q < NKEY; ++q)
+        skeys[q] = DENSE ? __builtin_amdgcn_readfirstlane(sample_key(skey, A.window_offset + wf + q))
+                         : sample_key(skey, A.window_offset + w0 + (rt0 >> 2) + q);
     }
 #pragma unroll
     for (int ct = 0; ct < NCT; ++ct) {
       const int co0 = (ct0 + ct) * 16 + 4 * h;
       const f32x4 b4 = gld<f32x4>(bias + co0);
       f32x4 s1 = {0.f, 0.f, 0.f, 0.f}, s2 = s1, k1 = s1, k0 = s1;
+      int mo = m;
+      if constexpr (DENSE) asm volatile("" : "+v"(mo));
 #pragma unroll
       for (int rt = 0; rt < NRT; ++rt) {
-        const int s = (rt0 + rt) >> 2, t = (((rt0 + rt) & 3) << 4) + m, w = w0 + s;
-        const bool valid = t < kL && w < A.n_win;
+        int t, w, sl = 0;
+        bool valid;
+        if constexpr (DENSE) {
+          const int dl = off + (rt0 + rt) * 16 + mo;
+          sl = dense::slot_of(dl), w = wf + sl, t = dl - sl * kL, valid = w < A.n_win;
+        } else {
+          const int s = (rt0 + rt) >> 2;
+          t = (((rt0 + rt) & 3) << 4) + m, w = w0 + s, valid = t < kL && w < A.n_win;
+        }
         f32x4 r;
 #pragma unroll
         for (int e = 0; e < 4; ++e) r[e] = fmaxf(__builtin_fmaf(acc[ct][rt][e], wsq[rt >> 2], b4[e]), 0.f);
         acc[ct][rt] = f32x4{0.f, 0.f, 0.f, 0.f};
         bool keep[4] = {true, true, true, true};
         if (drop) {
-          const unsigned key = skeys[rt >> 2];
+          unsigned key = skeys[DENSE ? 0 : rt >> 2];
+          if constexpr (DENSE) {
+#pragma unroll
+            for (int q = 1; q < NKEY; ++q) key = sl == q ? skeys[q] : key;
+          }
           const unsigned b01 = dropout_bits2(key, t, co0), b23 = dropout_bits2(key, t, co0 + 2);
           keep[0] = (b01 & 0xFFFFu) >= A.thr_out;
           keep[1] = (b01 >> 16) >= A.thr_out;
@@ -412,6 +467,7 @@
 
   const int total = (t_end - t_begin) * NCH;
   auto chunk_tile = [&](int it) { return t_begin + it / NCH; };
+  auto tile_off = [&](int tile) { return DENSE ? (int)((long long)(tile % tpg) * kRows % kL) : 0; };
   int g_cur = t_begin / tpg;
   if constexpr (LW > 0) {
     if (loader) {
@@ -452,7 +508,7 @@
       }
       const gf16x8* wcur = wbase(tile);
       const gf16x8* wnxt = wbase(tile + 1 < t_end ? tile + 1 : tile);
-      compute_chunk(c, smem + (it & 1) * kBufB, wcur, wnxt, []() {});
+      compute_chunk(c, tile_off(tile), smem + (it & 1) * kBufB, wcur, wnxt, []() {});
       if (c == NCH - 1) epilogue(tile);
       lds_barrier();
     }
@@ -480,7 +536,7 @@
     const gf16x8* wnxt = wbase(tile + 1 < t_end ? tile + 1 : tile);
     char* buf = smem + (it & 1) * kBufB;
     char* nbuf = smem + ((it + 1) & 1) * kBufB;
-    compute_chunk(c, buf, wcur, wnxt, [&]() {
+    compute_chunk(c, tile_off(tile), buf, wcur, wnxt, [&]() {
       if (stager && it + 1 < total) store_chunk(chunk_tile(it + 1), (it + 1) % NCH, nbuf, s0);
     });
     if (c == NCH - 1) epilogue(tile);
@@ -649,11 +705,11 @@
   }
 }
 
-template <int CIN, int COUT, int KS, int S, int WM, int WN, bool LAST, int LW, int CK, int WPC, bool PS>
+template <int CIN, int COUT, int KS, int S, int WM, int WN, bool LAST, int LW, int CK, int WPC, bool PS, bool DENSE = false>
 hipError_t launch_layer(const LayerArgs& A, int grid, hipStream_t stream) {
-  constexpr int lds = lds_bytes(S, COUT, CK);
+  constexpr int lds = lds_bytes(S, COUT, CK, DENSE);
   static_assert(WPC * lds <= 160 * 1024, "LDS of the workgroups sharing a CU");
-  auto k = layer_kernel<CIN, COUT, KS, S, WM, WN, LAST, LW, CK, WPC, PS>;
+  auto k = layer_kernel<CIN, COUT, KS, S, WM, WN, LAST, LW, CK, WPC, PS, DENSE>;
   static bool attr = false;
   if (!attr) {
     hipError_t e = hipFuncSetAttribute(reinterpret_cast<const void*>(k), hipFuncAttributeMaxDynamicSharedMemorySize, lds);
@@ -664,21 +720,30 @@
   return hipGetLastError();
 }
 
+template <bool HAVE, int CIN, int COUT, int KS, int S, int WM, int WN, int LW, int CK, int WPC>
+hipError_t launch_dense(const LayerArgs& A, int grid, hipStream_t stream) {
+  if constexpr (HAVE) {
+    return launch_layer<CIN, COUT, KS, S, WM, WN, false, (LW > 0 ? LW : -(WM * WN)), CK, WPC, false, true>(A, grid, stream);
+  } else {
+    return hipErrorInvalidValue;
+  }
+}
+
 }
 
 #ifdef APNEAUQ_X3_TABLE
 #include APNEAUQ_X3_TABLE
 #else
-#define APNEAUQ_X3_LAYERS(X)                     \
-  X(1, 128, 192, 5, 4, 2, 4, false, -8, 0, 32, 1) \
-  X(2, 192, 224, 3, 2, 1, 7, false, 4, 4, 64, 1) \
-  X(3, 224, 96, 7, 4, 2, 2, false, 4, 4, 32, 1)  \
-  X(4, 96, 256, 9, 2, 1, 8, false, 4, 4, 32, 1)  \
-  X(5, 256, 96, 9, 4, 2, 2, true, 4, 4, 64, 1)
+#define APNEAUQ_X3_LAYERS(X)                           \
+  X(1, 128, 192, 5, 4, 2, 4, false, -8, 0, 32, 1, true) \
+  X(2, 192, 224, 3, 2, 1, 7, false, 4, 4, 64, 1, true)  \
+  X(3, 224, 96, 7, 4, 2, 2, false, 4, 4, 32, 1, true)   \
+  X(4, 96, 256, 9, 2, 1, 8, false, 4, 4, 32, 1, true)   \
+  X(5, 256, 96, 9, 4, 2, 2, true, 4, 4, 64, 1, false)
 #endif
 
 int x3_lds_bytes(int layer) {
-#define APNEAUQ_X3_LDS(L, CI, CO, K, S, WM, WN, LAST, LW, LWB, CK, WPC) \
+#define APNEAUQ_X3_LDS(L, CI, CO, K, S, WM, WN, LAST, LW, LWB, CK, WPC, DENSE) \
   if (layer == L) return x3::lds_bytes(S, CO, CK);
   APNEAUQ_X3_LAYERS(APNEAUQ_X3_LDS)
 #undef APNEAUQ_X3_LDS
@@ -686,26 +751,37 @@
 }
 
 int x3_tile_samples(int layer) {
-#define APNEAUQ_X3_TS(L, CI, CO, K, S, WM, WN, LAST, LW, LWB, CK, WPC) \
+#define APNEAUQ_X3_TS(L, CI, CO, K, S, WM, WN, LAST, LW, LWB, CK, WPC, DENSE) \
   if (layer == L) return S;
   APNEAUQ_X3_LAYERS(APNEAUQ_X3_TS)
 #undef APNEAUQ_X3_TS
   return 0;
 }
 
+bool x3_has_dense(int layer) {
+#define APNEAUQ_X3_HD(L, CI, CO, K, S, WM, WN, LAST, LW, LWB, CK, WPC, DENSE) \
+  if (layer == L) return DENSE && !LAST;
+  APNEAUQ_X3_LAYERS(APNEAUQ_X3_HD)
+#undef APNEAUQ_X3_HD
+  return false;
+}
+
 int x3_wg_per_cu(int layer) {
-#define APNEAUQ_X3_WPC(L, CI, CO, K, S, WM, WN, LAST, LW, LWB, CK, WPC) \
+#define APNEAUQ_X3_WPC(L, CI, CO, K, S, WM, WN, LAST, LW, LWB, CK, WPC, DENSE) \
   if (layer == L) return WPC;
   APNEAUQ_X3_LAYERS(APNEAUQ_X3_WPC)
 #undef APNEAUQ_X3_WPC
   return 1;
 }
 
-hipError_t x3_launch_layer(int layer, const x3::LayerArgs& A, int grid, hipStream_t stream) {
+hipError_t x3_launch_layer(int layer, const x3::LayerArgs& A, int grid, bool dense_rows, hipStream_t stream) {
   using namespace x3;
   const bool ps = A.smax_in != nullptr || A.smax_out != nullptr;
-#define APNEAUQ_X3_LAUNCH(L, CI, CO, K, S, WM, WN, LAST, LW, LWB, CK, WPC)                                  \
+#define APNEAUQ_X3_LAUNCH(L, CI, CO, K, S, WM, WN, LAST, LW, LWB, CK, WPC, DENSE)                                  \
   if (layer == L) {                                                                                       \
+    if (dense_rows)                                                                                       \
+      return ps ? hipErrorInvalidValue                                                                    \
+                : launch_dense<DENSE && !LAST, CI, CO, K, S, WM, WN, LWB, CK, WPC>(A, grid, stream);       \
     return ps ? launch_layer<CI, CO, K, S, WM, WN, LAST, LW, CK, WPC, true>(A, grid, stream)               \
               : launch_layer<CI, CO, K, S, WM, WN, LAST, LWB, CK, WPC, false>(A, grid, stream);            \
   }
diff --git a/uncertaintyquantification_sleepapnea_1dcnn_amd/ops/x3.py b/uncertaintyquantification_sleepapnea_1dcnn_amd/ops/x3.py
--- a/uncertaintyquantification_sleepapnea_1dcnn_amd/ops/x3.py
+++ b/uncertaintyquantification_sleepapnea_1dcnn_amd/ops/x3.py
@@ -135,6 +135,24 @@
     return (l - 1) in sl and l >= 2, l in sl and l <= 4
 
 
+_DENSE_DEFAULT = "1,2,3,4"
+_dense_override: Optional[frozenset] = None
+
+
+def set_dense_layers(layers: Optional[Sequence[int]]) -> Optional[frozenset]:
+    global _dense_override
+    prev = _dense_override
+    _dense_override = None if layers is None else frozenset(int(l) for l in layers)
+    return prev
+
+
+def _dense_layers() -> frozenset:
+    if _dense_override is not None:
+        return _dense_override
+    v = os.environ.get("APNEAUQ_X3_DENSE", _DENSE_DEFAULT)
+    return frozenset(int(t) for t in v.replace(" ", "").split(",") if t)
+
+
 def _dsc(rate: float) -> float:
     return 1.0 / (1.0 - rate) if rate < 1.0 else 0.0
 
@@ -193,6 +211,7 @@
     eps, mom = float(spec.bn_epsilon), float(spec.bn_momentum)
     seed = int(seed) & ((1 << 63) - 1)
     sl = _sign_layers()
+    dl = _dense_layers()
     out = torch.empty(n_pass, n, dtype=torch.float32, device=model.device)
     ws.stats[0].zero_()
     o.x3_l1(x, model.w1, model.b1, ws.r1, ws.stats[0], n, 1, None)
@@ -212,7 +231,7 @@
             dst = ws.sums if l == 5 else ws.buf[(l - 1) % 2]
             o.x3_layer(l, src, dst, model.wfrag[l], 0, model.bias[l], model.wscale[l], 0, ws.aff[l - 1],
                        0 if l == 1 else 2 * CH[l], st, n, tc, l == 1, thr[l - 1], thr[l], seed, pb,
-                       int(window_offset), int(grid), None, None, None, ws.gscale[l - 1], *_sign(l, sl))
+                       int(window_offset), int(grid), None, None, None, ws.gscale[l - 1], *_sign(l, sl), l in dl)
             if sync is not None:
                 _sync_stats(sync, st, tc, c)
             g, b, mm, mv = model.bn[l]
@@ -237,6 +256,7 @@
     eps, mom = float(spec.bn_epsilon), float(spec.bn_momentum)
     seed = int(seed) & ((1 << 63) - 1)
     sl = _sign_layers()
+    dl = _dense_layers()
     out = torch.empty(n_pass, n, dtype=torch.float32, device=model.device)
 
     def run(s: int, e: int, upto: int, pb: int, stats_layer: int) -> None:
@@ -248,7 +268,7 @@
             o.x3_layer(l, src, dst, model.wfrag[l], 0, model.bias[l], model.wscale[l], 0, ws.aff[l - 1],
                        0 if l == 1 else 2 * CH[l], ws.stats[l] if l == stats_layer else None, m, 1, l == 1,
                        thr[l - 1], thr[l], seed, pb, int(window_offset) + s, 0, None, None, None, ws.gscale[l - 1],
-                       *_sign(l, sl))
+                       *_sign(l, sl), l in dl)
 
     def finish_layer(l: int, repeat: int) -> None:
         if sync is not None:
@@ -336,6 +356,7 @@
     n = x.shape[0]
     per_member = G > 1
     ps = CH[1:] if per_member else [0] * 6
+    dl = _dense_layers()
     o.zero_buffers([ws.stats[l][: G * STAT_SLOTS * 2 * CH[l + 1]] for l in range(5)])
     g, b, mm, mv = model.bn[5]
     o.x3_aff(None, g, b, mm, mv, ws.aff[5], CH[6], G, ps[5], False, 1, 1.0, eps, mom, 1.0, None)
@@ -349,7 +370,7 @@
         wstride = model.wfrag[l].shape[1] // 8 if per_member else 0
         o.x3_layer(l, src, dst, model.wfrag[l], wstride, model.bias[l], model.wscale[l], ps[l],
                    ws.aff[l - 1], 2 * CH[l] if per_member else 0, ws.stats[l] if l < 5 else None, n, G, False, 0, 0,
-                   0, 0, 0, 0, None, None, None, ws.gscale[l - 1], False, False)
+                   0, 0, 0, 0, None, None, None, ws.gscale[l - 1], False, False, l in dl)
     o.x3_head(ws.sums, ws.aff[5], 2 * CH[6] if per_member else 0, model.dw, model.db, CH[6] if per_member else 0,
               ws.out, n, G, bool(logits))
     return ws.out[: G * n].view(G, 1, n).clone()
```

Result: faster. 63400 windows/s (median of 6 runs) (+2.1%).
